# bdsaglam/torch-scae

Measured on AMD Instinct MI355X. Metric: images/sec SCAE fwd+bwd, MNIST 40x40 bs=128, 1/2/4/8 MI355X, higher is better.
Workload: dtype f32

## Files before the change

### include/scae_hip.h

```cpp
#ifndef SCAE_HIP_H
#define SCAE_HIP_H

#include <stdint.h>

#ifdef __cplusplus
extern "C" {
#endif

#define SCAE_ABI_VERSION 3

#define SCAE_OK 0
#define SCAE_ERR_BAD_ARG (-1)
#define SCAE_ERR_UNSUPPORTED (-2)

#define SCAE_MAX_CHANNELS 4
#define SCAE_ATTN_MAX_SET 64
#define SCAE_RENDER_MAX_TEMPLATE_ELEMS 4096

int scae_abi_version(void);
const char *scae_error_string(int code);

void *scae_launch_list_begin(void *stream);
int scae_launch_list_end(void *list);
int scae_launch_list_size(const void *list);
// ... 512 lines not shown

typedef struct scae_batch_source_desc {
  const void *images;
  const void *labels;
  const int32_t *index;
  int64_t rows;
  int64_t n;
  int image_u8, label_u8;
  int C, h, w, H, W;
  int shuffle, translate;
  uint64_t seed;
  int64_t epoch, position;
  int rank, world;
  int wrap;
  const int32_t *affine;
  int64_t affine_rows;
} scae_batch_source_desc;
int scae_gather_batch_f32(float *dst_image, int64_t *dst_label, int B,
                          const scae_batch_source_desc *src, void *stream);
int scae_step_prologue_source_f32(float *dst_image, int64_t *dst_label, int B,
                                  const scae_batch_source_desc *src, float *noise,
                                  int64_t n_noise, uint64_t *noise_state,
                                  const scae_seed_fold_desc *fold,
                                  const scae_first_layer_desc *first, void *stream);

int scae_template_color_supported(int M, int C, int F, int H1);
int scae_template_color_partial_rows(int B, int M);
int scae_template_color_fwd_f32(const float *logits, const float *feature, const float *w1,
                                const float *b1, const float *w2, const float *b2, float *raw,
                                float *templates, float *color, int B, int M, int C, int hw,
                                int F, int H1, int template_nonlin, int color_nonlin,
                                void *stream);
int scae_template_color_bwd_f32(const float *logits, const float *feature, const float *w1,
                                const float *b1, const float *w2, const float *b2,
                                const float *color, const float *g_templates,
                                const float *g_raw, float *g_logits, float *g_feature,
                                float *partial, int B, int M, int C, int hw, int F, int H1,
                                int template_nonlin, int color_nonlin, void *stream);

typedef struct scae_sum_segment {
  float *dst;
  int64_t begin, end, period;
} scae_sum_segment;
int scae_sum_rows_f32(const float *src, int64_t rows, int64_t cols,
                      const scae_sum_segment *segments, int n_segments, void *stream);
typedef struct scae_sum_job {
  const float *src;
  int64_t rows, cols;
  const scae_sum_segment *segments;
  int n_segments;
} scae_sum_job;
int scae_sum_rows_multi_f32(const scae_sum_job *jobs, int n_jobs, void *stream);

typedef struct scae_scaled_sum {
  const float *src;
  int64_t n;
  float scale;
  float *dst;
} scae_scaled_sum;
int scae_scaled_sums_f32(const scae_scaled_sum *jobs, int n_jobs, void *stream);

int scae_capsule_votes_fwd_f32(const float *all_param, const float *cpr_static,
                               const float *bias_cvr, const float *bias_caps,
                               const float *bias_vote, const float *bias_scale,
                               const float *noise_caps, const float *noise_vote,
                               float noise_scale, float *vote, float *scale,
                               float *vote_presence, float *logit_caps,
                               float *logit_vote, float *reg_partial,
                               float *caps_presence, int *caps_arg, int B, int O, int V,
                               int ld_param, int similarity, int learn_vote_scale,
                               int allow_deformations, void *stream);
int scae_capsule_votes_bwd_f32(const float *all_param, const float *cpr_static,
                               const float *bias_cvr, const float *bias_caps,
                               const float *bias_vote, const float *bias_scale,
                               const float *noise_caps, const float *noise_vote,
                               float noise_scale, const float *gvote,
                               const float *gscale, const float *gvote_presence,
                               const float *glogit_caps, const float *glogit_vote,
                               const float *greg, const float *gcaps_presence,
                               const int *caps_arg, float *gall_param, float *gcpr_in,
                               float *gall_param_gated, int B, int O, int V, int ld_param,
                               int similarity, int learn_vote_scale,
                               int allow_deformations, void *stream);

int scae_capsule_likelihood_fwd_f32(
    const float *vote, const float *scale, const float *vote_presence,
    const float *dummy_vote, const float *x, const float *presence,
    float *log_prob_per_point, float *vote_presence_binary, float *winner,
    float *winner_presence, int64_t *winner_idx, int64_t *is_from_capsule,
    float *soft_winner, float *soft_winner_presence, float *posterior,
    float *mixing_log_prob, float *mixing_logit, int B, int O, int M,
    void *stream);
int scae_capsule_likelihood_bwd_f32(
    const float *vote, const float *scale, const float *vote_presence,
    const float *dummy_vote, const float *x, const float *presence,
    const float *posterior, const int64_t *winner_idx, const float *g_lpp,
    const float *g_winner, const float *g_winner_presence,
    const float *g_soft_winner, const float *g_soft_winner_presence,
    const float *g_posterior, const float *g_mixing_log_prob,
    const float *g_mixing_logit, float *gvote, float *gscale,
    float *gvote_presence, float *gx, float *gpresence, float *gdummy_partial,
    int B, int O, int M, void *stream);

int scae_class_probs_supported(int O, int ncls);
int scae_class_probs_f32(const float *caps_presence, const float *posterior, const float *w,
                         const float *bias, float *prior_prob, float *post_prob, int B, int O,
                         int M, int ncls, const scae_scaled_sum *extra_sums, int n_extra,
                         void *stream);

typedef struct scae_eval_sink {
  float *rows;
  int64_t capacity;
  int64_t cursor;
  int64_t overflow;
} scae_eval_sink;
#define SCAE_EVAL_RECORD_FLOATS 9
#define SCAE_EVAL_RECORDS_MAX_CLASSES 64
typedef struct scae_eval_records {
  float *rows;
  int64_t capacity;
  int64_t cursor;
  int64_t overflow;
  int64_t *confusion;
  int64_t ncls;
  int64_t labelled;
} scae_eval_records;
#define SCAE_TRAIN_LOG_ROW 19
typedef struct scae_train_log_desc {
  float *rows;
  int64_t *step;
  int capacity;
  double *acc;
  const float *prior_prob, *post_prob;
  const int64_t *label;
  int ncls;
  const float *lr;
} scae_train_log_desc;
typedef struct scae_loss_extras {
  const float *rec_sums;
  int n_rec;
  const float *reg;
  float w_reg;
  float *g_rec_sums, *g_reg;
  float *loss;
  const float *g_loss;
  int defer_combine;
  float *out12;
  const scae_train_log_desc *train_log;
} scae_loss_extras;
int scae_loss_tail_supported(int B, int O, int ncls);
int64_t scae_loss_tail_workspace_floats(int B, int O, int ncls);
int scae_loss_tail_fwd_f32(const float *lpp, const float *posterior,
                           const float *caps_presence, const float *cls_w,
                           const float *cls_b, const int64_t *label,
                           const scae_loss_extras *extras, float *out12, float *workspace,
                           int B, int O, int M, int ncls, int n_classes_cfg, int prior_type,
                           int post_type, int sparsity_on, const float *weights5,
                           float within_const, void *stream);
int scae_loss_tail_defer_preferred(int B, int O);
int scae_loss_tail_combine_f32(const float *lpp, const float *posterior,
                               const float *caps_presence, const float *cls_w,
                               const float *cls_b, const int64_t *label,
                               const scae_loss_extras *extras, float *out12, float *workspace,
                               int B, int O, int M, int ncls, int n_classes_cfg, int prior_type,
                               int post_type, int sparsity_on, const float *weights5,
                               float within_const, void *stream);
int scae_loss_tail_fwd_class_probs_f32(
    const float *lpp, const float *posterior, const float *caps_presence, const float *cls_w,
    const float *cls_b, const int64_t *label, const scae_loss_extras *extras, float *out12,
    float *workspace, int B, int O, int M, int ncls, int n_classes_cfg, int prior_type,
    int post_type, int sparsity_on, const float *weights5, float within_const,
    const float *cp_caps_presence, const float *cp_posterior, const float *cp_w,
    const float *cp_bias, float *prior_prob, float *post_prob, int cp_B, int cp_O, int cp_M,
    int cp_ncls, const scae_scaled_sum *extra_sums, int n_extra, void *stream);
int scae_loss_tail_fwd_class_probs_sink_f32(
    const float *lpp, const float *posterior, const float *caps_presence, const float *cls_w,
    const float *cls_b, const int64_t *label, const scae_loss_extras *extras, float *out12,
    float *workspace, int B, int O, int M, int ncls, int n_classes_cfg, int prior_type,
    int post_type, int sparsity_on, const float *weights5, float within_const,
    const float *cp_caps_presence, const float *cp_posterior, const float *cp_w,
    const float *cp_bias, float *prior_prob, float *post_prob, int cp_B, int cp_O, int cp_M,
    int cp_ncls, const scae_scaled_sum *extra_sums, int n_extra, scae_eval_sink *sink,
    void *stream);
int scae_loss_tail_bwd_f32(const float *lpp, const float *posterior,
                           const float *caps_presence, const float *cls_w,
                           const float *cls_b, const int64_t *label,
                           const scae_loss_extras *extras, const float *gout12,
                           const float *workspace, float *g_lpp, float *g_posterior,
                           float *g_caps_presence, float *g_cls_w,
                           float *g_cls_b, int B, int O, int M, int ncls, int n_classes_cfg,
                           int prior_type, int post_type, int sparsity_on,
                           const float *weights5, float within_const, void *stream);

#define SCAE_EVAL_ACC_DOUBLES 17
int scae_eval_tail_f32(const float *lpp, const float *posterior, const float *caps_presence,
                       const float *cls_w, const float *cls_b, const int64_t *label,
                       const scae_loss_extras *extras, float *out12, float *workspace, int B,
                       int O, int M, int ncls, int n_classes_cfg, int prior_type,
                       int post_type, int sparsity_on, const float *weights5,
                       float within_const, const float *prior_prob, const float *post_prob,
                       double *acc, float *batch3, void *stream);
int scae_eval_tail_sink_f32(const float *lpp, const float *posterior, const float *caps_presence,
                            const float *cls_w, const float *cls_b, const int64_t *label,
                            const scae_loss_extras *extras, float *out12, float *workspace,
                            int B, int O, int M, int ncls, int n_classes_cfg, int prior_type,
                            int post_type, int sparsity_on, const float *weights5,
                            float within_const, const float *prior_prob, const float *post_prob,
                            double *acc, float *batch3, scae_eval_sink *sink, void *stream);
int scae_eval_tail_records_f32(const float *lpp, const float *posterior,
                               const float *caps_presence, const float *cls_w,
                               const float *cls_b, const int64_t *label,
                               const scae_loss_extras *extras, float *out12, float *workspace,
                               int B, int O, int M, int ncls, int n_classes_cfg, int prior_type,
                               int post_type, int sparsity_on, const float *weights5,
                               float within_const, const float *prior_prob,
                               const float *post_prob, double *acc, float *batch3,
                               scae_eval_sink *sink, scae_eval_records *records, void *stream);
int scae_eval_records_f32(const float *prior_prob, const float *post_prob, const int64_t *label,
                          const float *lpp, const float *rec_sums, const float *rec_pixels,
                          int B, int ncls, int M, int n_rec, scae_eval_records *records,
                          void *stream);
int scae_eval_accumulate_f32(const float *loss, const float *out12, const float *prior_prob,
                             const float *post_prob, const int64_t *label, int B, int ncls,
                             double *acc, float *batch3, void *stream);
int scae_eval_features_f32(const float *caps_presence, const float *posterior, int B, int O,
                           int M, scae_eval_sink *sink, void *stream);
int scae_train_log_f32(const float *loss, const float *out12, const float *extra2,
                       const scae_train_log_desc *log, int B, void *stream);

typedef struct scae_decoder_desc {
  const float *templates;
  const float *templates_alpha;
  const float *pose;
  const float *presence;
  const float *bg_image;
  const float *bg_value;
  const float *bg_mixing_logit;
  const float *temperature_logit;
  const float *out_scale;
  int B, M, C, th, tw, H, W;
  int template_repeat;
} scae_decoder_desc;

int scae_template_render_fwd_f32(const scae_decoder_desc *d,
                                 float *transformed_templates,
                                 float *mixing_logits, void *stream);

int scae_render_gmm_logprob_fwd_f32(const scae_decoder_desc *d, const float *x,
                                    float *log_prob, float *lse_post,
                                    float *lse_prior, void *stream);

int scae_render_gmm_bwd_f32(const scae_decoder_desc *d, const float *x,
                            const float *lse_post, const float *lse_prior,
                            const float *g_logprob, const float *g_tt,
                            const float *g_ml, float *g_templates,
                            float *g_alpha_partial, float *g_pose,
                            float *g_presence, float *g_bg_image,
                            float *g_scalar_partial, void *stream);
int scae_render_gmm_logprob_tiles(const scae_decoder_desc *d);
int scae_render_gmm_logprob_sums_fwd_f32(const scae_decoder_desc *d, const float *x,
                                         float *tile_sums, float *lse_post, float *lse_prior,
                                         void *stream);
int scae_render_gmm_sums_bwd_f32(const scae_decoder_desc *d, const float *x,
                                 const float *lse_post, const float *lse_prior,
                                 const float *g_tile_sums, float *g_templates,
                                 float *g_alpha_partial, float *g_pose, float *g_presence,
                                 float *g_bg_image, float *g_scalar_partial, void *stream);
#define SCAE_K1_FWD_WAVE 0
#define SCAE_K1_FWD_CLASSIC 1
#define SCAE_K1_RENDER_WAVE 0
#define SCAE_K1_RENDER_CLASSIC 1
#define SCAE_K1_BWD_CELL 0
#define SCAE_K1_BWD_SCATTER 1
#define SCAE_K1_BWD_GATHER 2
int scae_render_gmm_forms(const scae_decoder_desc *d, int fused, const void *tt,
                          const void *ml, int out[12]);


int scae_set_encoder_fwd_logprob_f32(int nseg, const float *const *seg_ptr,
                                     const int *seg_width, const int *seg_row_stride,
                                     const int64_t *seg_batch_stride, const float *presence,
                                     const float *params, float *z, float *hsave, int B, int N,
                                     int D, int Din, int Dout, int L, int layer_norm,
                                     const scae_decoder_desc *d, const float *x,
                                     float *tile_sums, float *lse_post, float *lse_prior,
                                     void *stream);

int scae_set_encoder_fwd_logprob_bf16(int nseg, const float *const *seg_ptr,
                                      const int *seg_width, const int *seg_row_stride,
                                      const int64_t *seg_batch_stride, const float *presence,
                                      const float *params, float *z, float *hsave, int B, int N,
                                      int D, int Din, int Dout, int L, int layer_norm,
                                      const scae_decoder_desc *d, const float *x,
                                      float *tile_sums, float *lse_post, float *lse_prior,
                                      void *stream);

typedef struct scae_likelihood_bwd_desc {
  const float *vote, *scale, *vote_presence, *dummy_vote, *x, *presence, *posterior;
  const int64_t *winner_idx;
  const float *g_lpp, *g_winner, *g_winner_presence, *g_soft_winner, *g_soft_winner_presence,
      *g_posterior, *g_mixing_log_prob, *g_mixing_logit;
  float *gvote, *gscale, *gvote_presence, *gx, *gpresence, *gdummy_partial;
  int B, O, M;
} scae_likelihood_bwd_desc;
int scae_render_gmm_sums_bwd_likelihood_f32(
    const scae_decoder_desc *d, const float *x, const float *lse_post, const float *lse_prior,
    const float *g_tile_sums, float *g_templates, float *g_alpha_partial, float *g_pose,
    float *g_presence, float *g_bg_image, float *g_scalar_partial,
    const scae_likelihood_bwd_desc *k, void *stream);

int scae_gmm_log_prob_fwd_f32(const float *loc, const float *mixing_logits,
                              const float *sigma, const float *x,
                              float *log_prob, int B, int K, int C, int Cm,
                              int64_t P, void *stream);
int scae_gmm_log_prob_bwd_f32(const float *loc, const float *mixing_logits,
                              const float *sigma, const float *x,
                              const float *g_logprob, float *g_loc,
                              float *g_ml, float *g_sigma_partial, float *g_x,
                              int B, int K, int C, int Cm, int64_t P,
                              void *stream);
int scae_gmm_mean_f32(const float *loc, const float *mixing_logits, float *out,
                      int B, int K, int C, int Cm, int64_t P, void *stream);
int scae_gmm_mode_f32(const float *loc, const float *mixing_logits,
                      const float *sigma, float *out, int maximum, int B,
                      int K, int C, int Cm, int64_t P, void *stream);

int scae_render_gmm_mode_f32(const scae_decoder_desc *d, float *out, int what, int first,
                             int count, void *stream);

int scae_render_gmm_parts_f32(const scae_decoder_desc *d, const float *x, const int *part_group,
                              const float *palette, int P, int *part, float *conf, float *mass,
                              float *mass_partial, int *group, float *rgb_part,
                              float *rgb_group, int first, int count, void *stream);
int scae_render_gmm_parts_geometry(const scae_decoder_desc *d, int count, int *out);

int scae_image_sheet_f32(int nsrc, const float *const *src, const int *n, int C, int H, int W,
                         int nrow, int padding, float pad_value, float *sheet, void *stream);

#define SCAE_KMEANS_MAX_K 256
#define SCAE_KMEANS_MAX_F 256
#define SCAE_KMEANS_MAX_KF 16384
#define SCAE_KMEANS_STATE_INTS 4
int scae_kmeans_supported(int k, int F);
int scae_kmeans_groups(int64_t N, int R);
typedef struct scae_kmeans_desc {
  const float *x;
  int64_t N;
  int F, k, R;
  int G;
  int max_iter;
  float *centroids;
  int64_t *labels;
  float *part_sum;
  int *part_count;
  int *part_changed;
  double *part_inertia;
  int *state;
  double *inertia;
} scae_kmeans_desc;
int scae_kmeans_lloyd_f32(const scae_kmeans_desc *d, int n_iters, void *stream);
int scae_kmeans_pp_f32(const float *x, int64_t N, int F, int k, int R, uint32_t seed,
                       float *centroids, float *d2, int64_t *chosen, void *stream);
int scae_kmeans_assign_f32(const float *x, int64_t N, int F, int k, const float *centroids,
                           int64_t *labels, void *stream);
int scae_kmeans_contingency(const int64_t *cluster_ids, const int64_t *labels, int64_t N, int k,
                            int ncls, int *table, int *outside, void *stream);

#define SCAE_PROBE_MAX_F 256
#define SCAE_PROBE_MAX_C 256
#define SCAE_PROBE_MAX_CF 16384
#define SCAE_PROBE_MAX_R 16
#define SCAE_PROBE_STATE_INTS 4
int scae_probe_supported(int F, int C, int R);
int scae_probe_groups(int64_t N, int F);
int scae_probe_predict_blocks(int64_t N);
int scae_probe_moments_f64(const float *x, const int64_t *y, int64_t N, int F, int C,
                           double *part, double *moments, int *outside, void *stream);
typedef struct scae_probe_desc {
  const float *x;
  const int64_t *y;
  int64_t N;
  int F, C, R;
  int G;
  int max_iter;
  const float *mean;
  const float *scale;
  const double *l2;
  const double *step;
  const double *tol;
  float *W, *V;
  float *grad;
  double *t;
  float *part_grad;
  double *part_loss;
  double *history;
  int *state;
} scae_probe_desc;
int scae_probe_fit_f32(const scae_probe_desc *d, int n_iters, void *stream);
int scae_probe_predict_f32(const float *x, int64_t N, int F, int C, const float *weight,
                           const float *bias, const int64_t *y, int64_t *pred, float *log_prob,
                           double *part_ce, double *mean_ce, void *stream);

#define SCAE_TSNE_MAX_N 32768
#define SCAE_TSNE_MAX_F 256
#define SCAE_TSNE_HISTORY_COLS 3
#define SCAE_TSNE_BLOCK_DOUBLES 640
int scae_tsne_supported(int N, int F);
int scae_tsne_groups(int N);
int scae_tsne_affinities_f32(const float *x, int N, int F, float perplexity, float *P,
                             float *beta, double *part, double *plogp, void *stream);
typedef struct scae_tsne_desc {
  int N;
  int G;
  int n_iter;
  int exaggeration_iter;
  int check_every;
  float early_exaggeration;
  float learning_rate;
  const float *P;
  float *Y, *velocity, *gains;
  float *part;
  float *rows;
  double *block;
  const double *plogp;
  double *history;
} scae_tsne_desc;
int scae_tsne_run_f32(const scae_tsne_desc *d, int first_iter, int n, void *stream);

#define SCAE_KNN_MAX_K 64
#define SCAE_KNN_MAX_F 256
#define SCAE_KNN_MAX_KS 8
int scae_knn_supported(int64_t Nq, int64_t Nb, int F, int k);
int scae_knn_groups(int64_t Nq, int64_t Nb);
int scae_knn_f32(const float *q, int64_t Nq, const float *base, int64_t Nb, int F, int k,
                 int self_mode, uint64_t *part, float *d2, int64_t *idx, void *stream);
int scae_knn_vote_f32(const int64_t *idx, const float *d2, int64_t Nq, int k,
                      const int64_t *base_labels, int64_t Nb, const int *ks, int n_ks,
                      int weighted, int64_t *pred, void *stream);
int scae_knn_ranks_f32(const float *x, int64_t N, int F, const int64_t *idx, int k, int *rank,
                       int *part_count, int64_t *part, int64_t *penalty, void *stream);

#define SCAE_TSNE_MAX_NEIGHBORS 128
#define SCAE_TSNE_SPARSE_MAX_N 262144
#define SCAE_TSNE_SPARSE_BLOCK_DOUBLES 5120
int scae_knn_wide_f32(const float *x, int64_t N, int F, int k, uint64_t *part, float *d2,
                      int64_t *idx, void *stream);
int scae_tsne_sparse_supported(int N, int F, int K);
int scae_tsne_sparse_groups(int N);
int scae_tsne_knn_bandwidths_f32(const float *d2, int N, int K, float perplexity, float *cond,
                                 float *beta, void *stream);
typedef struct scae_tsne_sparse_desc {
  int N;
  int G;
  int n_iter;
  int exaggeration_iter;
  int check_every;
  float early_exaggeration;
  float learning_rate;
  const int64_t *indptr;
  const int *cols;
  const float *vals;
  int64_t nnz;
  float *Y, *velocity, *gains;
  float *part;
  float *rows;
  double *block;
  const double *plogp;
  double *history;
} scae_tsne_sparse_desc;
int scae_tsne_sparse_run_f32(const scae_tsne_sparse_desc *d, int first_iter, int n, void *stream);

#define SCAE_CLUSTER_QUALITY_MAX_F 256
int scae_cluster_quality_supported(int64_t N, int F, int64_t k);
int scae_cluster_quality_labels(const int64_t *labels, int64_t N, int64_t k, int *lab32,
                                int *outside, void *stream);
int scae_cluster_quality_silhouette_f32(const float *xs, const int *ls, const int64_t *off,
                                        const int64_t *order, int64_t N, int F, int64_t k,
                                        double *values, double *a, double *b, int64_t *nearest,
                                        double *sorted_values, double *scores, void *stream);
int scae_cluster_quality_dispersion_f32(const float *xs, const int64_t *off, int64_t N, int F,
                                        int64_t k, double *table, void *stream);

#ifdef __cplusplus
}
#endif
#endif
```

### torch_scae_amd/_lib.py

```python
import ctypes
import os
from ctypes import c_float

from . import _abi

_HERE = os.path.dirname(os.path.abspath(__file__))
LIB_PATH = os.environ.get("SCAE_HIP_LIB") or os.path.join(_HERE, "lib",
                                                        "libscae_hip.so")
HEADER_PATH = os.path.join(os.path.dirname(_HERE), "include", "scae_hip.h")

DEVICE_STRUCTS = {"scae_eval_sink", "scae_eval_records"}


class ScaeHipError(RuntimeError):
    pass


def _read_header():
    if not os.path.exists(HEADER_PATH):
        raise ScaeHipError(
            f"{HEADER_PATH} is missing: the binding is derived from it, and torch_scae_amd "
            "runs from its source tree (restore the file, e.g. `git checkout "
            "include/scae_hip.h`).")
    with open(HEADER_PATH) as f:
        return _abi.parse(f.read(), by_address=DEVICE_STRUCTS)


ABI = _read_header()
SIGNATURES = {name: p.argtypes for name, p in ABI.prototypes.items()}
globals().update({cls.__name__: cls for cls in ABI.structs.values()})
globals().update({name[len("SCAE_"):]: value for name, value in ABI.defines.items()})
ABI_VERSION = ABI.defines["SCAE_ABI_VERSION"]
ERR_UNSUPPORTED = ABI.defines["SCAE_ERR_UNSUPPORTED"]

EVAL_SINK_INT64S = ctypes.sizeof(ABI.structs["scae_eval_sink"]) // 8
EVAL_RECORDS_INT64S = ctypes.sizeof(ABI.structs["scae_eval_records"]) // 8
assert (EVAL_SINK_INT64S, EVAL_RECORDS_INT64S) == (4, 7)
assert all(ctypes.sizeof(t) == 8 for name in DEVICE_STRUCTS
           for _, t in ABI.structs[name]._fields_)

_lib = None


def load():
    global _lib
    if _lib is not None:
        return _lib
    if not os.path.exists(LIB_PATH):
        raise ScaeHipError(
            f"{LIB_PATH} is missing: build it with `python -c 'import "
            f"__graft_entry__ as g; g.build()'` or `make -C torch_scae_amd/csrc`."
            " torch_scae_amd has no CPU / eager fallback.")
    lib = ctypes.CDLL(LIB_PATH)
    for name, proto in ABI.prototypes.items():
        fn = getattr(lib, name)
        fn.argtypes = proto.argtypes
        fn.restype = proto.restype
        if _is_launcher(proto):
            setattr(lib, name, _recording(fn))
    if lib.scae_abi_version() != ABI_VERSION:
        raise ScaeHipError(
            f"{LIB_PATH} has ABI version {lib.scae_abi_version()}, {HEADER_PATH} "
            f"declares version {ABI_VERSION}: rebuild it (make -C torch_scae_amd/csrc)")
    _lib = lib
    return lib


_RECORDER = None


def _is_launcher(proto):
    return (bool(proto.decls) and proto.decls[-1] == "void *stream"
            and not proto.name.startswith("scae_launch_list"))


def _recording(fn):
    def launcher(*args):
        rc = fn(*args)
        if _RECORDER is not None and rc == 0:
            conv = []
            for t, a in zip(fn.argtypes, args):
                if a is None or isinstance(a, (int, float)):
                    a = t(a) if a is not None else t()
                conv.append(a)
            _RECORDER.append((fn, tuple(conv[:-1]), args))
        return rc
    launcher.__name__ = getattr(fn, "__name__", "launcher")
    return launcher


class recorder:

    def __enter__(self):
        global _RECORDER
        self.prev, self.launches = _RECORDER, []
        _RECORDER = self.launches
        return self.launches

    def __exit__(self, *exc):
        global _RECORDER
        _RECORDER = self.prev
        return False


def replay(launches, stream):
    for fn, cargs, _keep in launches:
        rc = fn(*cargs, stream)
        if rc != 0:
            check(rc, getattr(fn, "__name__", "launch"))


def check(rc, what):
    if rc != 0:
        msg = load().scae_error_string(rc)
        raise ScaeHipError(f"{what} failed with code {rc}: "
                           f"{msg.decode() if msg else '?'}")


def call(name, *args):
    check(getattr(load(), name)(*args), name)


def try_call(name, *args):
    rc = getattr(load(), name)(*args)
    if rc == ERR_UNSUPPORTED:
        return False
    check(rc, name)
    return True
```

### torch_scae_amd/csrc/capsule_votes.hip

```cpp
#include "common.h"

#include "capsule_votes_dev.h"

namespace {
using namespace scae_votes;
constexpr int NT = 64;

__global__ __launch_bounds__(NT) void votes_fwd_kernel(
    VoteArgs a, float *__restrict__ vote, float *__restrict__ scale,
    float *__restrict__ vote_presence, float *__restrict__ logit_caps,
    float *__restrict__ logit_vote, float *__restrict__ reg_partial,
    float *__restrict__ caps_presence, int *__restrict__ caps_arg) {
  const int bo = blockIdx.x, o = bo % a.O, V = a.V, lane = threadIdx.x;
  const float *ap = a.all_param + (size_t)bo * a.ldp;

  float cv[6];
#pragma unroll
  for (int i = 0; i < 6; ++i) cv[i] = ap[6 * V + i] + a.bias_cvr[o * 6 + i];
  Xf C;
  xf_eval(cv, a.similarity, C);

  float lc = ap[6 * V + 6] + a.bias_caps[o];
  if (a.noise_caps) lc += (a.noise_caps[bo] - 0.5f) * a.noise_scale;
  const float pc = scae::sigmoidf_(lc);
  if (lane == 0) logit_caps[bo] = lc;

  float reg = 0.f;
  float best = -INFINITY;
  int best_v = 0x7fffffff;
  for (int v = lane; v < V; v += NT) {
    float pr[6];
#pragma unroll
    for (int i = 0; i < 6; ++i) {
      float dyn = a.allow_deformations ? ap[v * 6 + i] : 0.f;
      reg += dyn * dyn;
      pr[i] = dyn + a.cpr_static[((size_t)o * V + v) * 6 + i];
    }
    Xf P;
    xf_eval(pr, a.similarity, P);
    float *vo = vote + ((size_t)bo * V + v) * 6;
    vo[0] = C.o[0] * P.o[0] + C.o[1] * P.o[3];
    vo[1] = C.o[0] * P.o[1] + C.o[1] * P.o[4];
    vo[2] = C.o[0] * P.o[2] + C.o[1] * P.o[5] + C.o[2];
    vo[3] = C.o[3] * P.o[0] + C.o[4] * P.o[3];
    vo[4] = C.o[3] * P.o[1] + C.o[4] * P.o[4];
    vo[5] = C.o[3] * P.o[2] + C.o[4] * P.o[5] + C.o[5];

    float lv = ap[6 * V + 7 + v] + a.bias_vote[o * V + v];
    if (a.noise_vote) lv += (a.noise_vote[(size_t)bo * V + v] - 0.5f) * a.noise_scale;
    logit_vote[(size_t)bo * V + v] = lv;
    const float vpv = pc * scae::sigmoidf_(lv);
    vote_presence[(size_t)bo * V + v] = vpv;
    if (vpv > best) best = vpv, best_v = v;
    float sc = 1.f;
    if (a.learn_vote_scale)
      sc = scae::softplusf_(ap[7 * V + 7 + v] + a.bias_scale[o * V + v] + .5f) + 1e-2f;
    scale[(size_t)bo * V + v] = sc;
  }
  reg = scae::wave_sum(reg);
  if (lane == 0) reg_partial[bo] = reg;
  if (caps_presence) {
#pragma unroll
    for (int off = 32; off > 0; off >>= 1) {
      const float ov = __shfl_xor(best, off, 64);
      const int oi = __shfl_xor(best_v, off, 64);
      if (ov > best || (ov == best && oi < best_v)) best = ov, best_v = oi;
    }
    if (lane == 0) {
      caps_presence[bo] = best;
      caps_arg[bo] = best_v;
    }
  }
}

__global__ __launch_bounds__(NT) void votes_bwd_kernel(
    VoteArgs a, const float *__restrict__ gvote, const float *__restrict__ gscale,
    const float *__restrict__ gvp, const float *__restrict__ glc,
    const float *__restrict__ glv, const float *__restrict__ greg,
    float *__restrict__ gall, float *__restrict__ gcpr_in,
    const float *__restrict__ g_caps_presence, const int *__restrict__ caps_arg,
    float *__restrict__ gall_gated) {
  const int bo = blockIdx.x, o = bo % a.O, V = a.V, lane = threadIdx.x;
  const float *ap = a.all_param + (size_t)bo * a.ldp;
  float *ga = gall + (size_t)bo * a.ldp;
  float *gg = gall_gated ? gall_gated + (size_t)bo * a.ldp : nullptr;
  auto put = [&](int i, float v) {
    ga[i] = v;
    if (gg) gg[i] = ap[i] > 0.f ? v : 0.f;
  };

  float cv[6];
#pragma unroll
  for (int i = 0; i < 6; ++i) cv[i] = ap[6 * V + i] + a.bias_cvr[o * 6 + i];
  Xf C;
  xf_eval(cv, a.similarity, C);
  float lc = ap[6 * V + 6] + a.bias_caps[o];
  if (a.noise_caps) lc += (a.noise_caps[bo] - 0.5f) * a.noise_scale;
  const float pc = scae::sigmoidf_(lc);
  const float reg_w = greg ? greg[0] / (float)a.B : 0.f;

  float gC[6] = {0, 0, 0, 0, 0, 0};
  float gpc = 0.f;
  for (int v = lane; v < V; v += NT) {
    float pr[6], dyn[6];
#pragma unroll
    for (int i = 0; i < 6; ++i) {
      dyn[i] = a.allow_deformations ? ap[v * 6 + i] : 0.f;
      pr[i] = dyn[i] + a.cpr_static[((size_t)o * V + v) * 6 + i];
    }
    Xf P;
    xf_eval(pr, a.similarity, P);
    float gv[6] = {0, 0, 0, 0, 0, 0};
    if (gvote) {
#pragma unroll
      for (int i = 0; i < 6; ++i) gv[i] = gvote[((size_t)bo * V + v) * 6 + i];
    }
    gC[0] += gv[0] * P.o[0] + gv[1] * P.o[1] + gv[2] * P.o[2];
    gC[1] += gv[0] * P.o[3] + gv[1] * P.o[4] + gv[2] * P.o[5];
    gC[2] += gv[2];
    gC[3] += gv[3] * P.o[0] + gv[4] * P.o[1] + gv[5] * P.o[2];
    gC[4] += gv[3] * P.o[3] + gv[4] * P.o[4] + gv[5] * P.o[5];
    gC[5] += gv[5];
    float gP[6];
    gP[0] = gv[0] * C.o[0] + gv[3] * C.o[3];
    gP[1] = gv[1] * C.o[0] + gv[4] * C.o[3];
    gP[2] = gv[2] * C.o[0] + gv[5] * C.o[3];
    gP[3] = gv[0] * C.o[1] + gv[3] * C.o[4];
    gP[4] = gv[1] * C.o[1] + gv[4] * C.o[4];
    gP[5] = gv[2] * C.o[1] + gv[5] * C.o[4];
    float gin[6];
    xf_backward(P, a.similarity, gP, gin);
#pragma unroll
    for (int i = 0; i < 6; ++i) {
      gcpr_in[((size_t)bo * V + v) * 6 + i] = gin[i];
      put(v * 6 + i, a.allow_deformations ? gin[i] + reg_w * dyn[i] : 0.f);
    }

    float lv = ap[6 * V + 7 + v] + a.bias_vote[o * V + v];
    if (a.noise_vote) lv += (a.noise_vote[(size_t)bo * V + v] - 0.5f) * a.noise_scale;
    const float pv = scae::sigmoidf_(lv);
    float g_vp = gvp ? gvp[(size_t)bo * V + v] : 0.f;
    if (g_caps_presence && caps_arg[bo] == v) g_vp += g_caps_presence[bo];
    gpc += g_vp * pv;
    float g_lv = g_vp * pc * pv * (1.f - pv);
    if (glv) g_lv += glv[(size_t)bo * V + v];
    put(6 * V + 7 + v, g_lv);
    float g_sc = 0.f;
    if (a.learn_vote_scale && gscale)
      g_sc = gscale[(size_t)bo * V + v] *
             scae::softplus_grad(ap[7 * V + 7 + v] + a.bias_scale[o * V + v] + .5f);
    put(7 * V + 7 + v, g_sc);
  }
#pragma unroll
  for (int i = 0; i < 6; ++i) gC[i] = scae::wave_sum(gC[i]);
  gpc = scae::wave_sum(gpc);
  if (lane == 0) {
    float gin[6];
    xf_backward(C, a.similarity, gC, gin);
#pragma unroll
    for (int i = 0; i < 6; ++i) put(6 * V + i, gin[i]);
    float g_lc = gpc * pc * (1.f - pc);
    if (glc) g_lc += glc[bo];
    put(6 * V + 6, g_lc);
  }
}

int check_votes(const VoteArgs &a) {
  if (!a.all_param || !a.cpr_static || !a.bias_cvr || !a.bias_caps || !a.bias_vote ||
      !a.bias_scale)
    return SCAE_ERR_BAD_ARG;
  if (a.B <= 0 || a.O <= 0 || a.V <= 0 || a.ldp < 8 * a.V + 7) return SCAE_ERR_BAD_ARG;
  return SCAE_OK;
}
}

extern "C" int scae_capsule_votes_fwd_f32(
    const float *all_param, const float *cpr_static, const float *bias_cvr,
    const float *bias_caps, const float *bias_vote, const float *bias_scale,
    const float *noise_caps, const float *noise_vote, float noise_scale, float *vote,
    float *scale, float *vote_presence, float *logit_caps, float *logit_vote,
    float *reg_partial, float *caps_presence, int *caps_arg, int B, int O, int V,
    int ld_param, int similarity, int learn_vote_scale, int allow_deformations, void *stream) {
  VoteArgs a{all_param, cpr_static, bias_cvr, bias_caps, bias_vote, bias_scale,
             noise_caps, noise_vote, noise_scale, B, O, V, similarity, learn_vote_scale,
             allow_deformations, ld_param > 0 ? ld_param : 8 * V + 7};
  int rc = check_votes(a);
  if (rc) return rc;
  SCAE_REQUIRE(vote && scale && vote_presence && logit_caps && logit_vote && reg_partial);
  SCAE_REQUIRE(!caps_presence == !caps_arg);
  scae::launch(votes_fwd_kernel, dim3(B * O), dim3(NT), 0, (hipStream_t)stream, a,
                     vote, scale, vote_presence, logit_caps, logit_vote, reg_partial,
                     caps_presence, caps_arg);
  return scae_launch_status();
}

extern "C" int scae_capsule_votes_bwd_f32(
    const float *all_param, const float *cpr_static, const float *bias_cvr,
    const float *bias_caps, const float *bias_vote, const float *bias_scale,
    const float *noise_caps, const float *noise_vote, float noise_scale,
    const float *gvote, const float *gscale, const float *gvote_presence,
    const float *glogit_caps, const float *glogit_vote, const float *greg,
    const float *gcaps_presence, const int *caps_arg, float *gall_param, float *gcpr_in,
    float *gall_param_gated, int B, int O, int V, int ld_param, int similarity,
    int learn_vote_scale, int allow_deformations, void *stream) {
  VoteArgs a{all_param, cpr_static, bias_cvr, bias_caps, bias_vote, bias_scale,
             noise_caps, noise_vote, noise_scale, B, O, V, similarity, learn_vote_scale,
             allow_deformations, ld_param > 0 ? ld_param : 8 * V + 7};
  int rc = check_votes(a);
  if (rc) return rc;
  SCAE_REQUIRE(gall_param && gcpr_in && (!gcaps_presence || caps_arg));
  scae::launch(votes_bwd_kernel, dim3(B * O), dim3(NT), 0, (hipStream_t)stream, a,
                     gvote, gscale, gvote_presence, glogit_caps, glogit_vote, greg,
                     gall_param, gcpr_in, gcaps_presence, caps_arg, gall_param_gated);
  return scae_launch_status();
}
```

### torch_scae_amd/csrc/capsule_votes_dev.h

```cpp
#pragma once
#include "common.h"

namespace scae_votes {
constexpr float kTwoPi = 6.283185307179586f;

struct Xf {
  float sx, sy, sh, c, s, tx, ty;
  float dsx, dsy, dsh, dtx, dty;
  float o[6];
};

__device__ __forceinline__ void xf_eval(const float *p, int similarity, Xf &g) {
  const float ex = scae::sigmoidf_(p[0]), ey = scae::sigmoidf_(p[1]);
  g.sx = ex + 1e-2f;
  g.sy = ey + 1e-2f;
  g.dsx = ex * (1.f - ex);
  g.dsy = ey * (1.f - ey);
  g.sh = tanhf(p[3] * 5.f);
  g.tx = tanhf(p[4] * 5.f);
  g.ty = tanhf(p[5] * 5.f);
  g.dsh = 5.f * (1.f - g.sh * g.sh);
  g.dtx = 5.f * (1.f - g.tx * g.tx);
  g.dty = 5.f * (1.f - g.ty * g.ty);
  const float th = p[2] * kTwoPi;
  g.c = cosf(th);
  g.s = sinf(th);
  if (similarity) {
    g.o[0] = g.sx * g.c;
    g.o[1] = -g.sx * g.s;
    g.o[2] = g.tx;
    g.o[3] = g.sx * g.s;
    g.o[4] = g.sx * g.c;
    g.o[5] = g.ty;
  } else {
    g.o[0] = g.sx * g.c + g.sh * g.sy * g.s;
    g.o[1] = -g.sx * g.s + g.sh * g.sy * g.c;
    g.o[2] = g.tx;
    g.o[3] = g.sy * g.s;
    g.o[4] = g.sy * g.c;
    g.o[5] = g.ty;
  }
}

__device__ __forceinline__ void xf_backward(const Xf &g, int similarity, const float *go,
                                            float *gp) {
  float gsx, gsy, gsh, gth;
  if (similarity) {
    gsx = go[0] * g.c - go[1] * g.s + go[3] * g.s + go[4] * g.c;
    gsy = 0.f;
    gsh = 0.f;
    gth = g.sx * (-go[0] * g.s - go[1] * g.c + go[3] * g.c - go[4] * g.s);
  } else {
    gsx = go[0] * g.c - go[1] * g.s;
    gsy = go[0] * g.sh * g.s + go[1] * g.sh * g.c + go[3] * g.s + go[4] * g.c;
    gsh = go[0] * g.sy * g.s + go[1] * g.sy * g.c;
    gth = go[0] * (-g.sx * g.s + g.sh * g.sy * g.c) +
          go[1] * (-g.sx * g.c - g.sh * g.sy * g.s) + go[3] * g.sy * g.c - go[4] * g.sy * g.s;
  }
  gp[0] = gsx * g.dsx;
  gp[1] = gsy * g.dsy;
  gp[2] = gth * kTwoPi;
  gp[3] = gsh * g.dsh;
  gp[4] = go[2] * g.dtx;
  gp[5] = go[5] * g.dty;
}

struct VoteArgs {
  const float *all_param, *cpr_static, *bias_cvr, *bias_caps, *bias_vote, *bias_scale;
  const float *noise_caps, *noise_vote;
  float noise_scale;
  int B, O, V, similarity, learn_vote_scale, allow_deformations;
  int ldp;
};


struct VoteOut {
  float *vote, *scale, *vote_presence, *logit_caps, *logit_vote, *reg_partial, *caps_presence;
  int *caps_arg;
};
struct VoteGrads {
  const float *gvote, *gscale, *gvp, *glc, *glv, *greg, *g_caps_presence;
  const int *caps_arg;
  float *gall, *gcpr_in, *gall_gated;
};

template <int NTH>
__device__ __forceinline__ void fwd_block(const VoteArgs &a, const VoteOut &w, const float *rows,
                                          int ld, float *red, int b0, int o) {
  const int V = a.V, tid = threadIdx.x;
  for (int e = tid; e < 16 * V; e += NTH) {
    const int i = e / V, v = e - i * V, b = b0 + i;
    const float *ap = rows + i * ld;
    float regv = 0.f, vpv = -INFINITY;
    if (b < a.B) {
      const int bo = b * a.O + o;
      float cv[6];
#pragma unroll
      for (int k = 0; k < 6; ++k) cv[k] = ap[6 * V + k] + a.bias_cvr[o * 6 + k];
      Xf C;
      xf_eval(cv, a.similarity, C);
      float lc = ap[6 * V + 6] + a.bias_caps[o];
      if (a.noise_caps) lc += (a.noise_caps[bo] - 0.5f) * a.noise_scale;
      const float pc = scae::sigmoidf_(lc);
      if (v == 0) w.logit_caps[bo] = lc;
      float pr[6];
#pragma unroll
      for (int k = 0; k < 6; ++k) {
        const float dyn = a.allow_deformations ? ap[v * 6 + k] : 0.f;
        regv += dyn * dyn;
        pr[k] = dyn + a.cpr_static[((size_t)o * V + v) * 6 + k];
      }
      Xf P;
      xf_eval(pr, a.similarity, P);
      float *vo = w.vote + ((size_t)bo * V + v) * 6;
      vo[0] = C.o[0] * P.o[0] + C.o[1] * P.o[3];
      vo[1] = C.o[0] * P.o[1] + C.o[1] * P.o[4];
      vo[2] = C.o[0] * P.o[2] + C.o[1] * P.o[5] + C.o[2];
      vo[3] = C.o[3] * P.o[0] + C.o[4] * P.o[3];
      vo[4] = C.o[3] * P.o[1] + C.o[4] * P.o[4];
      vo[5] = C.o[3] * P.o[2] + C.o[4] * P.o[5] + C.o[5];
      float lv = ap[6 * V + 7 + v] + a.bias_vote[o * V + v];
      if (a.noise_vote) lv += (a.noise_vote[(size_t)bo * V + v] - 0.5f) * a.noise_scale;
      w.logit_vote[(size_t)bo * V + v] = lv;
      vpv = pc * scae::sigmoidf_(lv);
      w.vote_presence[(size_t)bo * V + v] = vpv;
      float sc = 1.f;
      if (a.learn_vote_scale)
        sc = scae::softplusf_(ap[7 * V + 7 + v] + a.bias_scale[o * V + v] + .5f) + 1e-2f;
      w.scale[(size_t)bo * V + v] = sc;
    }
    red[e] = regv;
    red[16 * V + e] = vpv;
  }
  __syncthreads();
  if (tid < 256) {
    const int i = tid >> 4, l = tid & 15;
    float reg = 0.f, best = -INFINITY;
    int best_v = 0x7fffffff;
    for (int v = l; v < V; v += 16) {
      reg += red[i * V + v];
      const float p = red[16 * V + i * V + v];
      if (p > best) best = p, best_v = v;
    }
#pragma unroll
    for (int off = 8; off > 0; off >>= 1) {
      reg += __shfl_xor(reg, off, 64);
      const float ov = __shfl_xor(best, off, 64);
      const int oi = __shfl_xor(best_v, off, 64);
      if (ov > best || (ov == best && oi < best_v)) best = ov, best_v = oi;
    }
    if (l == 0 && b0 + i < a.B) {
      const int bo = (b0 + i) * a.O + o;
      w.reg_partial[bo] = reg;
      if (w.caps_presence) {
        w.caps_presence[bo] = best;
        w.caps_arg[bo] = best_v;
      }
    }
  }
}

template <int NTH>
__device__ __forceinline__ void bwd_block(const VoteArgs &a, const VoteGrads &w, float *grows,
                                          int ld, float *red, int b0, int o) {
  const int V = a.V, tid = threadIdx.x, A = 8 * V + 7;
  const float reg_w = w.greg ? w.greg[0] / (float)a.B : 0.f;
  auto put = [&](const float *ap, int i, int bo, int col, float v) {
    w.gall[(size_t)bo * a.ldp + col] = v;
    const float gv = ap[col] > 0.f ? v : 0.f;
    if (w.gall_gated) w.gall_gated[(size_t)bo * a.ldp + col] = gv;
    grows[i * ld + col] = w.gall_gated ? gv : v;
  };
  for (int e = tid; e < 16 * V; e += NTH) {
    const int i = e / V, v = e - i * V, b = b0 + i;
    float part[7] = {0.f, 0.f, 0.f, 0.f, 0.f, 0.f, 0.f};
    if (b < a.B) {
      const int bo = b * a.O + o;
      const float *ap = a.all_param + (size_t)bo * a.ldp;
      float cv[6];
#pragma unroll
      for (int k = 0; k < 6; ++k) cv[k] = ap[6 * V + k] + a.bias_cvr[o * 6 + k];
      Xf C;
      xf_eval(cv, a.similarity, C);
      float lc = ap[6 * V + 6] + a.bias_caps[o];
      if (a.noise_caps) lc += (a.noise_caps[bo] - 0.5f) * a.noise_scale;
      const float pc = scae::sigmoidf_(lc);
      float pr[6], dyn[6];
#pragma unroll
      for (int k = 0; k < 6; ++k) {
        dyn[k] = a.allow_deformations ? ap[v * 6 + k] : 0.f;
        pr[k] = dyn[k] + a.cpr_static[((size_t)o * V + v) * 6 + k];
      }
      Xf P;
      xf_eval(pr, a.similarity, P);
      float gv[6] = {0, 0, 0, 0, 0, 0};
      if (w.gvote) {
#pragma unroll
        for (int k = 0; k < 6; ++k) gv[k] = w.gvote[((size_t)bo * V + v) * 6 + k];
      }
      part[0] = gv[0] * P.o[0] + gv[1] * P.o[1] + gv[2] * P.o[2];
      part[1] = gv[0] * P.o[3] + gv[1] * P.o[4] + gv[2] * P.o[5];
      part[2] = gv[2];
      part[3] = gv[3] * P.o[0] + gv[4] * P.o[1] + gv[5] * P.o[2];
      part[4] = gv[3] * P.o[3] + gv[4] * P.o[4] + gv[5] * P.o[5];
      part[5] = gv[5];
      float gP[6];
      gP[0] = gv[0] * C.o[0] + gv[3] * C.o[3];
      gP[1] = gv[1] * C.o[0] + gv[4] * C.o[3];
      gP[2] = gv[2] * C.o[0] + gv[5] * C.o[3];
      gP[3] = gv[0] * C.o[1] + gv[3] * C.o[4];
      gP[4] = gv[1] * C.o[1] + gv[4] * C.o[4];
      gP[5] = gv[2] * C.o[1] + gv[5] * C.o[4];
      float gin[6];
      xf_backward(P, a.similarity, gP, gin);
#pragma unroll
      for (int k = 0; k < 6; ++k) {
        w.gcpr_in[((size_t)bo * V + v) * 6 + k] = gin[k];
        put(ap, i, bo, v * 6 + k, a.allow_deformations ? gin[k] + reg_w * dyn[k] : 0.f);
      }
      float lv = ap[6 * V + 7 + v] + a.bias_vote[o * V + v];
      if (a.noise_vote) lv += (a.noise_vote[(size_t)bo * V + v] - 0.5f) * a.noise_scale;
      const float pv = scae::sigmoidf_(lv);
      float g_vp = w.gvp ? w.gvp[(size_t)bo * V + v] : 0.f;
      if (w.g_caps_presence && w.caps_arg[bo] == v) g_vp += w.g_caps_presence[bo];
      part[6] = g_vp * pv;
      float g_lv = g_vp * pc * pv * (1.f - pv);
      if (w.glv) g_lv += w.glv[(size_t)bo * V + v];
      put(ap, i, bo, 6 * V + 7 + v, g_lv);
      float g_sc = 0.f;
      if (a.learn_vote_scale && w.gscale)
        g_sc = w.gscale[(size_t)bo * V + v] *
               scae::softplus_grad(ap[7 * V + 7 + v] + a.bias_scale[o * V + v] + .5f);
      put(ap, i, bo, 7 * V + 7 + v, g_sc);
    }
#pragma unroll
    for (int k = 0; k < 7; ++k) red[(size_t)e * 7 + k] = part[k];
  }
  __syncthreads();
  {
    float t = 0.f;
    const int i = tid >> 5, k = (tid >> 2) & 7, part = tid & 3;
    if (tid < 512 && k < 7)
      for (int v = part; v < V; v += 4) t += red[(size_t)(i * V + v) * 7 + k];
    t += __shfl_xor(t, 1, 64);
    t += __shfl_xor(t, 2, 64);
    __syncthreads();
    if (tid < 512 && k < 7 && part == 0) red[i * 8 + k] = t;
  }
  __syncthreads();
  if (tid < 16) {
    const int i = tid, b = b0 + i;
    if (b < a.B) {
      const int bo = b * a.O + o;
      const float *ap = a.all_param + (size_t)bo * a.ldp;
      float gC[6], gpc = red[i * 8 + 6];
#pragma unroll
      for (int k = 0; k < 6; ++k) gC[k] = red[i * 8 + k];
      float cv[6];
#pragma unroll
      for (int k = 0; k < 6; ++k) cv[k] = ap[6 * V + k] + a.bias_cvr[o * 6 + k];
      Xf C;
      xf_eval(cv, a.similarity, C);
      float lc = ap[6 * V + 6] + a.bias_caps[o];
      if (a.noise_caps) lc += (a.noise_caps[bo] - 0.5f) * a.noise_scale;
      const float pc = scae::sigmoidf_(lc);
      float gin[6];
      xf_backward(C, a.similarity, gC, gin);
#pragma unroll
      for (int k = 0; k < 6; ++k) put(ap, i, bo, 6 * V + k, gin[k]);
      float g_lc = gpc * pc * (1.f - pc);
      if (w.glc) g_lc += w.glc[bo];
      put(ap, i, bo, 6 * V + 6, g_lc);
    } else {
      for (int col = 0; col < A; ++col) grows[i * ld + col] = 0.f;
    }
  }
  const int a16 = (A + 15) & ~15;
  for (int e = tid; e < 16 * (a16 - A); e += NTH) {
    const int i = e / (a16 - A), col = A + e - i * (a16 - A);
    grows[i * ld + col] = 0.f;
  }
  __syncthreads();
}
}
```

### torch_scae_amd/csrc/render_bwd_likelihood.hip

```cpp
#include "common.h"
#include "capsule_likelihood_dev.h"
#include "render_gmm_wave_dev.h"

namespace {
struct LkBwd {
  scae_lk::LkArgs a;
  const int64_t *winner_idx;
  const float *g_lpp, *g_winner, *g_winner_presence, *g_soft_winner, *g_soft_winner_presence,
      *g_posterior, *g_mlp, *g_mlogit;
  float *gvote, *gscale, *gvp, *gx, *gpresence, *gdummy;
};

template <int C>
__global__ __launch_bounds__(256, 5) void bwd_cell_likelihood_kernel(
    scae_decoder_desc d, const float *__restrict__ x, const float *__restrict__ lse_post,
    const float *__restrict__ lse_prior, const float *__restrict__ g_tile, int lp_tiles,
    int lp_ppb, float *__restrict__ g_templates, float *__restrict__ g_alpha_partial,
    float *__restrict__ g_pose, float *__restrict__ g_presence, float *__restrict__ g_bg_image,
    float *__restrict__ g_scalar_partial, int chunk_rows, int max_items, int item_budget,
    LkBwd lk, int n_lk) {
  extern __shared__ __attribute__((aligned(16))) float smem[];
  if ((int)blockIdx.x < n_lk) {
    scae_lk::likelihood_bwd_body<false, 256>(
        lk.a, lk.winner_idx, lk.g_lpp, lk.g_winner, lk.g_winner_presence, lk.g_soft_winner,
        lk.g_soft_winner_presence, lk.g_posterior, lk.g_mlp, lk.g_mlogit, lk.gvote, lk.gscale,
        lk.gvp, lk.gx, lk.gpresence, lk.gdummy, smem, blockIdx.x, n_lk);
    return;
  }
  const int id = (int)blockIdx.x - n_lk, K = d.M + 1, b = id / K, k = id - b * K;
  scae_k1::bwd_cell_body<C, 256>(d, x, lse_post, lse_prior, nullptr, g_tile, lp_tiles, lp_ppb,
                                 g_templates, g_alpha_partial, g_pose, g_presence, g_bg_image,
                                 g_scalar_partial, chunk_rows, max_items, item_budget, smem, k, b);
}

template <int C>
int launch(const scae_decoder_desc *d, const scae_k1::CellGeom &g, const scae_k1::LpTiling &lt,
           const float *x, const float *lse_post, const float *lse_prior, const float *g_tile,
           float *g_templates, float *g_alpha_partial, float *g_pose, float *g_presence,
           float *g_bg_image, float *g_scalar_partial, const LkBwd &lk, hipStream_t st) {
  const size_t lds_k = scae_lk::lk_lds(lk.a.O, lk.a.M, true);
  const size_t lds = g.lds > lds_k ? g.lds : lds_k;
  if (lds > 48 * 1024) {
    hipError_t e =
        hipFuncSetAttribute(reinterpret_cast<const void *>(bwd_cell_likelihood_kernel<C>),
                            hipFuncAttributeMaxDynamicSharedMemorySize, (int)lds);
    if (e != hipSuccess) return (int)e;
  }
  const int n_lk = lk.a.B < 1024 ? lk.a.B : 1024;
  scae::launch((bwd_cell_likelihood_kernel<C>), dim3(n_lk + (d->M + 1) * d->B), dim3(256),
                     lds, st, *d, x, lse_post, lse_prior, g_tile, lt.tiles, lt.ppb, g_templates,
                     g_alpha_partial, g_pose, g_presence, g_bg_image, g_scalar_partial,
                     g.chunk_rows, g.max_items, g.item_budget, lk, n_lk);
  return scae_launch_status();
}
}

extern "C" int scae_render_gmm_sums_bwd_likelihood_f32(
    const scae_decoder_desc *d, const float *x, const float *lse_post, const float *lse_prior,
    const float *g_tile_sums, float *g_templates, float *g_alpha_partial, float *g_pose,
    float *g_presence, float *g_bg_image, float *g_scalar_partial,
    const scae_likelihood_bwd_desc *k, void *stream) {
  SCAE_REQUIRE(d && k);
  const char *e = getenv("SCAE_FUSE_K1_K4_BWD");
  const scae_k1::CellGeom g = scae_k1::cell_geom(d);
  const bool fits = !(e && *e == '0') && g.lds && (d->C == 1 || d->C == 3) && k->O <= 64 &&
                    scae_lk::lk_lds(k->O, k->M, true) <= g.lds && k->B > 0 && k->O > 0 &&
                    k->M > 0 && d->template_repeat <= 1;
  if (!fits) {
    int rc = scae_render_gmm_sums_bwd_f32(d, x, lse_post, lse_prior, g_tile_sums, g_templates,
                                          g_alpha_partial, g_pose, g_presence, g_bg_image,
                                          g_scalar_partial, stream);
    if (rc) return rc;
    return scae_capsule_likelihood_bwd_f32(
        k->vote, k->scale, k->vote_presence, k->dummy_vote, k->x, k->presence, k->posterior,
        k->winner_idx, k->g_lpp, k->g_winner, k->g_winner_presence, k->g_soft_winner,
        k->g_soft_winner_presence, k->g_posterior, k->g_mixing_log_prob, k->g_mixing_logit,
        k->gvote, k->gscale, k->gvote_presence, k->gx, k->gpresence, k->gdummy_partial, k->B,
        k->O, k->M, stream);
  }
  SCAE_REQUIRE(x && lse_post && lse_prior && g_tile_sums && g_templates && g_alpha_partial &&
               g_pose && g_scalar_partial);
  SCAE_REQUIRE(k->vote && k->scale && k->vote_presence && k->dummy_vote && k->x &&
               k->posterior && k->winner_idx && k->gvote && k->gscale && k->gvote_presence &&
               k->gx && k->gdummy_partial);
  const scae_k1::LpTiling lt = scae_k1::lp_tiling(d);
  LkBwd lk{{k->vote, k->scale, k->vote_presence, k->dummy_vote, k->x, k->presence, k->B, k->O,
            k->M},
           k->winner_idx,
           k->g_lpp,
           k->g_winner,
           k->g_winner_presence,
           k->g_soft_winner,
           k->g_soft_winner_presence,
           k->g_posterior,
           k->g_mixing_log_prob,
           k->g_mixing_logit,
           k->gvote,
           k->gscale,
           k->gvote_presence,
           k->gx,
           k->gpresence,
           k->gdummy_partial};
  hipStream_t st = (hipStream_t)stream;
  return d->C == 1 ? launch<1>(d, g, lt, x, lse_post, lse_prior, g_tile_sums, g_templates,
                               g_alpha_partial, g_pose, g_presence, g_bg_image, g_scalar_partial,
                               lk, st)
                   : launch<3>(d, g, lt, x, lse_post, lse_prior, g_tile_sums, g_templates,
                               g_alpha_partial, g_pose, g_presence, g_bg_image, g_scalar_partial,
                               lk, st);
}
```

### torch_scae_amd/ops.py

```python
import collections
import ctypes
import functools

import numpy as np
import torch

from . import _lib, step_plan
from ._lib import DecoderDesc, ScaeHipError
from .step_plan import StepPlan, current as _plan

__all__ = ["geometric_transform", "qkv_attention", "set_encoder", "grouped_mlp", "seed_attention", "seed_attention_supported", "seed_fold", "seed_fold_supported", "loss_tail", "loss_tail_scalar", "loss_tail_supported", "capsule_votes",
           "capsule_likelihood", "colored_templates", "template_color_supported", "attention_conv_pool", "attention_pool_supported", "capsule_head", "part_encoder", "conv_stack", "conv_stack_supported",
           "uniform", "reset_noise", "pack_params", "render_templates", "render_gmm_log_prob", "render_gmm_log_prob_sums",
           "gmm_log_prob", "gmm_mean", "gmm_mode", "render_gmm_mode", "render_gmm_parts", "GmmParts", "image_sheet", "ScaeHipError"]


def _need_hip(*tensors):
    for t in tensors:
        if t is None:
            continue
        if not t.is_cuda:
            raise ScaeHipError(
                "torch_scae_amd ops run only on a HIP device (got a "
                f"{t.device} tensor); there is no CPU path.")
# ... 1790 lines not shown
            gy2 = gy2.contiguous()
        gw = _grad_out(ctx.slots[0], weight)
        gb = _grad_out(ctx.slots[1], weight, (N,)) if ctx.has_bias else None
        wgrad = _gemm_desc(_p(gy2), _p(x2), _p(gw), 1, N, K, M, False, N, 0,
                           False, K, 0, K, 0, asum=_p(gb), asum_b=0, asum_ld=1)
        if ctx.needs_input_grad[0]:
            gx = torch.empty(M, K, device=x2.device, dtype=x2.dtype)
            dgrad = _gemm_desc(_p(gy2), _p(weight), _p(gx), 1, M, K, N, True, N,
                               0, False, K, 0, K, 0)
            _gemm_pair(wgrad, dgrad, x2)
            gx = gx.view(ctx.x_shape)
        else:
            gx = None
            _lib.call("scae_gemm_multi_f32", (_lib.GemmDesc * 1)(wgrad), 1,
                      _stream(x2))
        return gx, gw, gb


def linear(x, weight, bias=None):
    return _Linear.apply(x, weight, bias)


class HipLinear(torch.nn.Linear):

    def forward(self, x):
        if x.is_cuda and x.dtype == torch.float32 and \
                self.weight.dtype == torch.float32 and not _bf16() and \
                not torch.is_autocast_enabled("cuda"):
            return linear(x, self.weight, self.bias)
        return torch.nn.functional.linear(x, self.weight, self.bias)


class _LayerNorm(torch.autograd.Function):

    @_fwd
    def forward(ctx, x, weight, bias, eps):
        _need_hip(x, weight, bias)
        d = x.shape[-1]
        x2 = x.reshape(-1, d).contiguous()
        rows = x2.shape[0]
        y = torch.empty_like(x2)
        mean = torch.empty(rows, device=x.device, dtype=x.dtype)
        rstd = torch.empty_like(mean)
        _lib.call("scae_layer_norm_fwd_f32", _p(x2), _p(_c(weight)),
                  _p(_c(bias)), _p(y), _p(mean), _p(rstd), rows, d, float(eps),
                  _stream(x))
        ctx.save_for_backward(x2, mean, rstd, *([weight] if weight is not None
                                                else []))
        ctx.has = (weight is not None, bias is not None)
        ctx.x_shape = x.shape
        ctx.slots = (_slot(weight, ctx) if weight is not None else None,
                     _slot(bias, ctx) if bias is not None else None)
        return y.view(x.shape)

    @_bwd
    def backward(ctx, gy):
        x2, mean, rstd = ctx.saved_tensors[:3]
        weight = ctx.saved_tensors[3] if ctx.has[0] else None
        rows, d = x2.shape
        gy2 = gy.reshape(rows, d).contiguous()
        gx = torch.empty_like(x2) if ctx.needs_input_grad[0] else None
        want_p = ctx.has[0] or ctx.has[1]
        partial = torch.empty(_lib.load().scae_layer_norm_rows(rows), 2 * d,
                              device=x2.device, dtype=x2.dtype) \
            if want_p else None
        _lib.call("scae_layer_norm_bwd_f32", _p(x2), _p(_c(weight)), _p(mean),
                  _p(rstd), _p(gy2), _p(gx), _p(partial), rows, d, _stream(x2))
        gw = gb = None
        if want_p:
            outs = [_grad_out(ctx.slots[0], x2, (d,)) if ctx.has[0] else
                    torch.empty(d, device=x2.device, dtype=x2.dtype),
                    _grad_out(ctx.slots[1], x2, (d,)) if ctx.has[1] else
                    torch.empty(d, device=x2.device, dtype=x2.dtype)]
            gw, gb = _sum_rows(partial, [(d,), (d,)], outs=outs)
            gw = gw if ctx.has[0] else None
            gb = gb if ctx.has[1] else None
        return (None if gx is None else gx.view(ctx.x_shape)), gw, gb, None


class HipLayerNorm(torch.nn.LayerNorm):

    def forward(self, x):
        if x.is_cuda and x.dtype == torch.float32 and \
                len(self.normalized_shape) == 1 and \
                self.normalized_shape[0] <= 1024 and \
                not torch.is_autocast_enabled("cuda"):
            return _LayerNorm.apply(x, self.weight, self.bias, self.eps)
        return super().forward(x)


def mlp_chain_supported(x, layers):
    if not x.is_cuda or x.dtype != torch.float32 or \
            not 1 <= len(layers) <= 4:
        return False
    wmax = _lib.load().scae_mlp_chain_max_width()
    return x.shape[2] <= wmax and all(
        w.shape[1] <= wmax and w.shape[2] <= wmax + 1 and
        not (ones and b is not None) for w, b, ones in layers)


def _chain_forward_desc(x, ones_flags, weights, biases):
    L = len(ones_flags)
    B, G, Kin = x.shape
    d = _lib.MlpChainDesc()
    d.n_layers, d.in_, d.in_gs, d.in_bs, d.in_dim, d.B, d.G = \
        L, x.data_ptr(), x.stride(1), x.stride(0), Kin, B, G
    d.row_tile = _CHAIN_ROW_TILE
    d.bf16 = int(_bf16())
    acts, K = [], Kin
    for l, (w, b) in enumerate(zip(weights, biases)):
        N, ldw = w.shape[1], w.shape[2]
        assert ldw == K + (1 if ones_flags[l] else 0)
        if l == L - 1:
            Np = (N + 3) // 4 * 4
            out = torch.empty(B, G, Np, device=x.device,
                              dtype=x.dtype)[:, :, :N]
            out_gs, out_bs = Np, G * Np
        else:
            out = torch.empty(G, B, N, device=x.device, dtype=x.dtype)
            out_gs, out_bs = B * N, N
        y = d.layer[l]
        y.w, y.w_gs, y.ldw, y.K, y.N = w.data_ptr(), N * ldw, ldw, K, N
        if ones_flags[l]:
            y.bias, y.bias_gs, y.bias_ld = w.data_ptr() + 4 * K, N * ldw, ldw
        elif b is not None:
            y.bias, y.bias_gs, y.bias_ld = b.data_ptr(), N, 1
        y.out, y.out_gs, y.out_bs, y.relu = out.data_ptr(), out_gs, out_bs, 1
        acts.append(out)
        K = N
    return d, acts


_CHAIN_ROW_TILE = 0


def _chain_backward(x, weights, acts, ones_flags, has_bias, x_is_relu, slots,
                    need_gx, gpre=None, votes=None, park=False):
    L = len(ones_flags)
    B, G, Kin = x.shape
    dev, dt = x.device, x.dtype
    d = _lib.MlpChainDesc()
    d.n_layers, d.in_, d.in_gs, d.in_bs, d.in_dim, d.B, d.G = \
        L, gpre.data_ptr(), gpre.stride(1), gpre.stride(0), gpre.shape[2], B, G
    d.row_tile = _CHAIN_ROW_TILE
    d.bf16 = int(_bf16())
    gx = torch.empty(B, G, Kin, device=dev, dtype=dt) if need_gx else None
    gs = [None] * L
    gs[L - 1] = gpre
    n_chain = 0
    for i, l in enumerate(range(L - 1, -1, -1)):
        w = weights[l]
        N, ldw = w.shape[1], w.shape[2]
        K = ldw - (1 if ones_flags[l] else 0)
        if l == 0 and not need_gx:
            break
        y = d.layer[i]
        y.w, y.w_gs, y.ldw, y.K, y.N = w.data_ptr(), N * ldw, ldw, N, K
        if l > 0:
            gs[l - 1] = torch.empty(G, B, K, device=dev, dtype=dt)
            y.gate, y.gate_gs, y.gate_bs = acts[l - 1].data_ptr(), B * K, K
            y.out, y.out_gs, y.out_bs = gs[l - 1].data_ptr(), B * K, K
        else:
            if x_is_relu:
                y.gate, y.gate_gs, y.gate_bs = x.data_ptr(), x.stride(1), \
                    x.stride(0)
            y.out, y.out_gs, y.out_bs = gx.data_ptr(), K, G * K
        n_chain += 1
    d.n_layers = n_chain
    if votes is not None:
        assert n_chain >= 1
        _lib.call("scae_mlp_chain_votes_bwd_f32", ctypes.byref(d),
                  ctypes.byref(votes), _stream(x))
    elif n_chain:
        _lib.call("scae_mlp_chain_bwd_f32", ctypes.byref(d), _stream(x))
    descs = (_lib.GemmDesc * L)()
    gws, gbs = [None] * L, [None] * L
    for l in range(L):
        w = weights[l]
        N, ldw = w.shape[1], w.shape[2]
        K = ldw - (1 if ones_flags[l] else 0)
        if l == 0:
            xin, x_ld, x_b = x, x.stride(0), x.stride(1)
        else:
            xin, x_ld, x_b = acts[l - 1], K, B * K
        g = gs[l]
        if l == L - 1:
            g_ld, g_b = g.stride(0), g.stride(1)
        else:
            g_ld, g_b = N, B * N
        gw = _grad_out(slots[l], w)
        asum_ld = 1
        if has_bias[l]:
            gsum = _grad_out(slots[L + l], w, (G, N))
            asum, asum_b = _p(gsum), N
            gbs[l] = gsum
        elif ones_flags[l]:
            asum, asum_b, asum_ld = _off(gw, K), N * ldw, ldw
        else:
            asum, asum_b = None, 0
        descs[l] = _gemm_desc(_p(g), _p(xin), _p(gw), G, N, K, B, False,
                              g_ld, g_b, False, x_ld, x_b, ldw, N * ldw,
                              asum=asum, asum_b=asum_b, asum_ld=asum_ld)
        gws[l] = gw
    if park and not _bf16() and L <= 4 and all(_in_slot(t) for t in gws) and \
            all(_in_slot(t) for t in gbs if t is not None):
        _plan().park("wgrads", _PendingWeightGemms(
            descs, L, (x, gs, acts, [w for w in weights]), x))
    else:
        _lib.call(_prec("scae_gemm_multi_f32"), descs, L, _stream(x))
    return gx, gws, gbs


class _MLPChain(torch.autograd.Function):

    @_fwd
    def forward(ctx, x, ones_flags, x_is_relu, *wb):
        L = len(ones_flags)
        _need_hip(x, *wb)
        if x.stride(2) != 1:
            x = x.contiguous()
        weights = [w.contiguous() for w in wb[:L]]
        biases = [None if b is None else b.contiguous() for b in wb[L:]]
        d, acts = _chain_forward_desc(x, ones_flags, weights, biases)
        _lib.call("scae_mlp_chain_fwd_f32", ctypes.byref(d), _stream(x))
        ctx.save_for_backward(x, *weights, *acts)
        ctx.meta = (tuple(ones_flags), [b is not None for b in biases],
                    bool(x_is_relu))
        ctx.slots = [_slot(t, ctx) for t in wb]
        return acts[-1]

    @_bwd
    def backward(ctx, gy):
        ones_flags, has_bias, x_is_relu = ctx.meta
        L = len(ones_flags)
        x = ctx.saved_tensors[0]
        weights = ctx.saved_tensors[1:1 + L]
        acts = ctx.saved_tensors[1 + L:]
        G = x.shape[1]
        gpre = gy
        if not (gpre.stride(2) == 1 and gpre.stride(1) >= gpre.shape[2]
                and gpre.stride(0) == G * gpre.stride(1)):
            gpre = gpre.contiguous()
        gx, gws, gbs = _chain_backward(x, weights, acts, ones_flags, has_bias,
                                       x_is_relu, ctx.slots,
                                       ctx.needs_input_grad[0], gpre=gpre)
        return (gx, None, None, *gws, *gbs)


class _ChainVotes(torch.autograd.Function):

    @_fwd
    def forward(ctx, x, ones_flags, vflags, noise_scale, cpr_static, b_cvr,
                b_caps, b_vote, b_scale, noise_caps, noise_vote, *wb):
        L = len(ones_flags)
        similarity, learn_vote_scale, allow_deformations, defer_reg = vflags
        _need_hip(x, cpr_static, b_cvr, b_caps, b_vote, b_scale, noise_caps,
                  noise_vote, *wb)
        if x.stride(2) != 1:
            x = x.contiguous()
        weights = [w.contiguous() for w in wb[:L]]
        biases = [None if b is None else b.contiguous() for b in wb[L:]]
        vargs = [_c(t) for t in (cpr_static, b_cvr, b_caps, b_vote, b_scale,
                                 noise_caps, noise_vote)]
        d, acts = _chain_forward_desc(x, ones_flags, weights, biases)
        all_param = acts[-1]
        B, O, A = all_param.shape
        V, ldp = (A - 7) // 8, all_param.stride(1)
        assert A == 8 * V + 7
        dev, dt = x.device, x.dtype
        new = lambda *shape: torch.empty(*shape, device=dev, dtype=dt)
        vote, scale, vp = new(B, O, V, 6), new(B, O, V), new(B, O, V)
        lc, lv, reg = new(B, O, 1), new(B, O, V), new(B, O)
        reg_loss = torch.empty((), device=dev, dtype=dt)
        caps_presence = new(B, O)
        caps_arg = torch.empty(B, O, device=dev, dtype=torch.int32)
        v = _lib.VotesDesc()
        for name, t in zip(("cpr_static", "bias_cvr", "bias_caps", "bias_vote",
                            "bias_scale", "noise_caps", "noise_vote"), vargs):
            setattr(v, name, None if t is None else t.data_ptr())
        v.noise_scale, v.V, v.ld_param = float(noise_scale), V, ldp
        v.similarity, v.learn_vote_scale, v.allow_deformations = \
            int(similarity), int(learn_vote_scale), int(allow_deformations)
        for name, t in (("vote", vote), ("scale", scale), ("vote_presence", vp),
                        ("logit_caps", lc), ("logit_vote", lv),
                        ("reg_partial", reg), ("caps_presence", caps_presence),
                        ("caps_arg", caps_arg)):
            setattr(v, name, t.data_ptr())
        _lib.call("scae_mlp_chain_votes_fwd_f32", ctypes.byref(d),
                  ctypes.byref(v), _stream(x))
        if not defer_reg:
            scaled_sums([(reg, 0.5 / B, reg_loss)])
        ctx.save_for_backward(x, caps_arg, *weights, *acts,
                              *[t for t in vargs if t is not None])
        ctx.has_noise = (vargs[5] is not None, vargs[6] is not None)
        ctx.meta = (tuple(ones_flags), [b is not None for b in biases],
                    float(noise_scale), (V, ldp, int(similarity),
                                         int(learn_vote_scale),
                                         int(allow_deformations)))
        ctx.slots = [_slot(t, ctx) for t in wb]
        ctx.vslots = [_slot(t, ctx) for t in (cpr_static, b_cvr, b_caps, b_vote,
                                         b_scale)]
        ctx.set_materialize_grads(False)
        ctx.mark_non_differentiable(reg)
        return vote, scale, vp, lc, lv, reg_loss, caps_presence, reg

    @_bwd
    def backward(ctx, gvote, gscale, gvp, glc, glv, greg, gcp, _greg_partial):
        ones_flags, has_bias, noise_scale, (V, ldp, sim, lvs, adef) = ctx.meta
        L = len(ones_flags)
        saved = list(ctx.saved_tensors)
        x, caps_arg = saved[0], saved[1]
        weights = saved[2:2 + L]
        acts = saved[2 + L:2 + 2 * L]
        rest = saved[2 + 2 * L:]
        vargs = rest[:5]
        rest = rest[5:]
        noise_caps = rest.pop(0) if ctx.has_noise[0] else None
        noise_vote = rest.pop(0) if ctx.has_noise[1] else None
        all_param = acts[-1]
        B, O, A = all_param.shape
        dev, dt = x.device, x.dtype
        padded = lambda: torch.empty(B, O, ldp, device=dev,
                                     dtype=dt)[:, :, :A]
        gall, ggated = padded(), padded()
        gin = torch.empty(B, O, V, 6, device=dev, dtype=dt)
        grads = [_c(g) for g in (gvote, gscale, gvp, glc, glv, greg, gcp)]
        v = _lib.VotesDesc()
        for name, t in zip(("all_param", "cpr_static", "bias_cvr", "bias_caps",
                            "bias_vote", "bias_scale", "noise_caps",
                            "noise_vote"),
                           [all_param, *vargs, noise_caps, noise_vote]):
            setattr(v, name, None if t is None else t.data_ptr())
        v.noise_scale, v.V, v.ld_param = noise_scale, V, ldp
        v.similarity, v.learn_vote_scale, v.allow_deformations = sim, lvs, adef
        for name, t in zip(("gvote", "gscale", "gvote_presence", "glogit_caps",
                            "glogit_vote", "greg", "gcaps_presence"), grads):
            setattr(v, name, None if t is None else t.data_ptr())
        v.caps_arg = caps_arg.data_ptr()
        v.gall_param, v.gcpr_in, v.gall_param_gated = \
            gall.data_ptr(), gin.data_ptr(), ggated.data_ptr()
        gx, gws, gbs = _chain_backward(
            x, weights, acts, ones_flags, has_bias, False, ctx.slots, True,
            gpre=ggated, votes=v,
            park=ctx.plan.parking)
        outs = [_grad_out(sl, t) for sl, t in zip(ctx.vslots, vargs)]
        gall_rows = torch.as_strided(gall, (B, O * ldp), (O * ldp, 1))
        (g_static,), (g_cvr, g_caps, g_vote, g_scale) = _sum_rows_multi([
            dict(partial=gin.view(B, -1), shapes=[vargs[0].shape],
                 outs=outs[:1], defer=ctx.vslots[0] is not None),
            dict(partial=gall_rows, shapes=[t.shape for t in vargs[1:5]],
                 starts=[6 * V, 6 * V + 6, 6 * V + 7, 7 * V + 7], period=ldp,
                 outs=outs[1:],
                 defer=all(sl is not None for sl in ctx.vslots[1:5]))])
        return (gx, None, None, None, g_static, g_cvr, g_caps, g_vote, g_scale,
                None, None, *gws, *gbs)


def chain_votes(x, layers, cpr_static, bias_cvr, bias_caps, bias_vote,
                bias_scale, noise_caps=None, noise_vote=None, noise_scale=0.,
                similarity=False, learn_vote_scale=True,
                allow_deformations=True, defer_reg=False):
    ws = [w for w, _, _ in layers]
    bs = [b for _, b, _ in layers]
    return _ChainVotes.apply(
        x, tuple(bool(o) for _, _, o in layers),
        (bool(similarity), bool(learn_vote_scale), bool(allow_deformations),
         bool(defer_reg)), float(noise_scale), cpr_static, bias_cvr, bias_caps,
        bias_vote, bias_scale, noise_caps, noise_vote, *ws, *bs)


def mlp_chain(x, layers, x_is_relu=False):
    ws = [w for w, _, _ in layers]
    bs = [b for _, b, _ in layers]
    return _MLPChain.apply(x, tuple(bool(o) for _, _, o in layers),
                           bool(x_is_relu), *ws, *bs)


def grouped_mlp(x, weights, biases, ones_input=False, grad_pregated=False,
                x_is_relu=False, pad_out=False):
    biases = list(biases) if biases is not None else [None] * len(weights)
    return _GroupedMLP.apply(x, ones_input, len(weights), grad_pregated,
                             x_is_relu, pad_out, *weights, *biases)


class _CapsuleVotes(torch.autograd.Function):
    @_fwd
    def forward(ctx, all_param, cpr_static, b_cvr, b_caps, b_vote, b_scale,
                noise_caps, noise_vote, noise_scale, similarity,
                learn_vote_scale, allow_deformations, param_is_relu,
                defer_reg):
        _need_hip(all_param, cpr_static, b_cvr, b_caps, b_vote, b_scale,
                  noise_caps, noise_vote)
        B, O, A = all_param.shape
        V = (A - 7) // 8
        ldp = all_param.stride(1)
        if not (all_param.stride(2) == 1 and ldp >= A
                and all_param.stride(0) == O * ldp):
            all_param, ldp = all_param.contiguous(), A
        args = [all_param] + [_c(t) for t in (cpr_static, b_cvr, b_caps, b_vote,
                                              b_scale, noise_caps, noise_vote)]
        dev, dt = all_param.device, all_param.dtype
        vote = torch.empty(B, O, V, 6, device=dev, dtype=dt)
        scale = torch.empty(B, O, V, device=dev, dtype=dt)
        vp = torch.empty(B, O, V, device=dev, dtype=dt)
        lc = torch.empty(B, O, 1, device=dev, dtype=dt)
        lv = torch.empty(B, O, V, device=dev, dtype=dt)
        reg = torch.empty(B, O, device=dev, dtype=dt)
        reg_loss = torch.empty((), device=dev, dtype=dt)
        caps_presence = torch.empty(B, O, device=dev, dtype=dt)
        caps_arg = torch.empty(B, O, device=dev, dtype=torch.int32)
        flags = (B, O, V, ldp, int(similarity), int(learn_vote_scale),
                 int(allow_deformations))
        _lib.call("scae_capsule_votes_fwd_f32", *[_p(t) for t in args],
                  float(noise_scale), _p(vote), _p(scale), _p(vp), _p(lc),
                  _p(lv), _p(reg), _p(caps_presence), _p(caps_arg), *flags,
                  _stream(all_param))
        if not defer_reg:
            scaled_sums([(reg, 0.5 / B, reg_loss)])
        ctx.save_for_backward(caps_arg, *[t for t in args if t is not None])
        ctx.has_noise = (args[6] is not None, args[7] is not None)
        ctx.noise_scale = float(noise_scale)
        ctx.flags = flags
        ctx.param_is_relu = bool(param_is_relu)
        ctx.slots = [_slot(t, ctx) for t in (cpr_static, b_cvr, b_caps, b_vote,
                                        b_scale)]
        ctx.set_materialize_grads(False)
        ctx.mark_non_differentiable(reg)
        return vote, scale, vp, lc, lv, reg_loss, caps_presence, reg

    @_bwd
    def backward(ctx, gvote, gscale, gvp, glc, glv, greg, gcp, _greg_partial):
        saved = list(ctx.saved_tensors)
        caps_arg = saved.pop(0)
        args = saved[:6]
        args.append(saved.pop(6) if ctx.has_noise[0] else None)
        args.append(saved[6] if ctx.has_noise[1] else None)
        all_param = args[0]
        B, O, V, ldp = ctx.flags[:4]
        A = all_param.shape[2]
        padded = lambda: torch.empty(B, O, ldp, device=all_param.device,
                                     dtype=all_param.dtype)[:, :, :A]
        gall = padded()
        ggated = padded() if ctx.param_is_relu else None
        gin = torch.empty(B, O, V, 6, device=all_param.device,
                          dtype=all_param.dtype)
        grads = [_c(g) for g in (gvote, gscale, gvp, glc, glv, greg, gcp)]
        _lib.call("scae_capsule_votes_bwd_f32", *[_p(t) for t in args],
                  ctx.noise_scale, *[_p(g) for g in grads], _p(caps_arg),
                  _p(gall), _p(gin), _p(ggated), *ctx.flags,
                  _stream(all_param))
        outs = [_grad_out(sl, t) for sl, t in zip(ctx.slots, args[1:6])]
        gall_rows = torch.as_strided(gall, (B, O * ldp), (O * ldp, 1))
        (g_static,), (g_cvr, g_caps, g_vote, g_scale) = _sum_rows_multi([
            dict(partial=gin.view(B, -1), shapes=[args[1].shape],
                 outs=outs[:1], defer=ctx.slots[0] is not None),
            dict(partial=gall_rows,
                 shapes=[t.shape for t in args[2:6]],
                 starts=[6 * V, 6 * V + 6, 6 * V + 7, 7 * V + 7], period=ldp,
                 outs=outs[1:],
                 defer=all(sl is not None for sl in ctx.slots[1:5]))])
        return (gall if ggated is None else ggated, g_static, g_cvr, g_caps,
                g_vote, g_scale, None, None, None, None, None, None, None, None)


def capsule_votes(all_param, cpr_static, bias_cvr, bias_caps, bias_vote,
                  bias_scale, noise_caps=None, noise_vote=None, noise_scale=0.,
                  similarity=False, learn_vote_scale=True,
                  allow_deformations=True, param_is_relu=False,
                  defer_reg=False):
    return _CapsuleVotes.apply(all_param, cpr_static, bias_cvr, bias_caps,
                               bias_vote, bias_scale, noise_caps, noise_vote,
                               noise_scale, similarity, learn_vote_scale,
                               allow_deformations, param_is_relu, defer_reg)


class _CapsuleLikelihood(torch.autograd.Function):
    @_fwd
    def forward(ctx, vote, scale, vp, dummy_vote, x, presence, defer_sum):
        _need_hip(vote, scale, vp, dummy_vote, x, presence)
        vote, scale, vp, dummy_vote, x, presence = (
            _c(t) for t in (vote, scale, vp, dummy_vote, x, presence))
        B, O, M, _ = vote.shape
        dev, dt = vote.device, vote.dtype
        f = lambda *s: torch.empty(*s, device=dev, dtype=dt)
        lpp, binary = f(B, M), f(B, O, M)
        winner, winner_p = f(B, M, 6), f(B, M)
        widx = torch.empty(B, M, device=dev, dtype=torch.int64)
        from_caps = torch.empty(B, M, device=dev, dtype=torch.int64)
        soft, soft_p = f(B, M, 6), f(B, M)
        post, mlp, mlogit = f(B, O + 1, M), f(B, O + 1, M), f(B, O + 1, M)
        log_prob = torch.empty((), device=dev, dtype=dt)
        _lib.call("scae_capsule_likelihood_fwd_f32", _p(vote), _p(scale),
                  _p(vp), _p(dummy_vote), _p(x), _p(presence), _p(lpp),
                  _p(binary), _p(winner), _p(winner_p), _p(widx),
                  _p(from_caps), _p(soft), _p(soft_p), _p(post), _p(mlp),
                  _p(mlogit), B, O, M, _stream(vote))
        if not defer_sum:
            scaled_sums([(lpp, 1.0 / B, log_prob)])
        saved = [vote, scale, vp, dummy_vote, x, post, widx]
        if presence is not None:
            saved.append(presence)
        ctx.save_for_backward(*saved)
        ctx.has_presence = presence is not None
        ctx.dims = (B, O, M)
        ctx.dummy_shape = dummy_vote.shape
        ctx.mark_non_differentiable(binary, widx, from_caps)
        ctx.set_materialize_grads(False)
        return (lpp, binary, winner, winner_p, widx, from_caps, soft, soft_p,
                post, mlp, mlogit, log_prob)

    @_bwd
    def backward(ctx, g_lpp, _gb, g_w, g_wp, _gi, _gf, g_s, g_sp, g_post,
                 g_mlp, g_mlogit, g_log_prob):
        saved = ctx.saved_tensors
        vote, scale, vp, dummy_vote, x, post, widx = saved[:7]
        presence = saved[7] if ctx.has_presence else None
        B, O, M = ctx.dims
        if g_log_prob is not None:
            spread = (g_log_prob / B).expand(B, M)
            g_lpp = spread if g_lpp is None else g_lpp + spread
        gvote, gscale, gvp = (torch.empty_like(t) for t in (vote, scale, vp))
        gx = torch.empty_like(x)
        gpres = torch.empty(B, M, device=x.device, dtype=x.dtype) \
            if presence is not None else None
        gdummy = torch.empty(B, M, 6, device=x.device, dtype=x.dtype)
        gin = [_c(g) for g in (g_lpp, g_w, g_wp, g_s, g_sp, g_post, g_mlp,
                               g_mlogit)]
        pending = ctx.plan.take("k1_bwd")
        if pending is not None and any(
                g is not None for g in (g_w, g_wp, g_s, g_sp)):
            pending.launch_alone()
            pending = None
        if pending is not None and pending.ref.device == vote.device:
            k = _lib.LikelihoodBwdDesc()
            for name, t in zip(
                    ("vote", "scale", "vote_presence", "dummy_vote", "x",
                     "presence", "posterior", "winner_idx", "g_lpp",
                     "g_winner", "g_winner_presence", "g_soft_winner",
                     "g_soft_winner_presence", "g_posterior",
                     "g_mixing_log_prob", "g_mixing_logit", "gvote", "gscale",
                     "gvote_presence", "gx", "gpresence", "gdummy_partial"),
                    (vote, scale, vp, dummy_vote, x, presence, post, widx,
                     *gin, gvote, gscale, gvp, gx, gpres, gdummy)):
                setattr(k, name, None if t is None else t.data_ptr())
            k.B, k.O, k.M = B, O, M
            _lib.call("scae_render_gmm_sums_bwd_likelihood_f32",
                      ctypes.byref(pending.desc), *pending.ptrs,
                      ctypes.byref(k), _stream(vote))
        else:
            if pending is not None:
                pending.launch_alone()
            _lib.call("scae_capsule_likelihood_bwd_f32", _p(vote), _p(scale),
                      _p(vp), _p(dummy_vote), _p(x), _p(presence), _p(post),
                      _p(widx), *[_p(g) for g in gin], _p(gvote), _p(gscale),
                      _p(gvp), _p(gx), _p(gpres), _p(gdummy), B, O, M,
                      _stream(vote))
        g_dummy = None
        if g_w is not None or g_s is not None:
            g_dummy = _sum_rows(gdummy.view(B, -1), [ctx.dummy_shape])[0]
        return gvote, gscale, gvp, g_dummy, gx, gpres, None


def capsule_likelihood(vote, scale, vote_presence, dummy_vote, x,
                       presence=None, defer_sum=False):
    return _CapsuleLikelihood.apply(vote, scale, vote_presence, dummy_vote, x,
                                    presence, defer_sum)


_SPARSITY_TYPES = {"l2": 0, "entropy": 1, "kl": 2}


def loss_tail_supported(B, O, n_classes):
    return bool(_lib.load().scae_loss_tail_supported(B, O, n_classes or 0))


class _LossTail(torch.autograd.Function):
    @_fwd
    def forward(ctx, lpp, posterior, caps_presence, cls_w, cls_b, label,
                rec_sums, reg, cfg):
        _need_hip(lpp, posterior, caps_presence, cls_w, cls_b, rec_sums, reg)
        ctx.slots = (_slot(cls_w, ctx), _slot(cls_b, ctx))
        lpp, posterior, caps_presence = _c(lpp), _c(posterior), _c(caps_presence)
        cls_w, cls_b, label = _c(cls_w), _c(cls_b), _c(label)
        rec_sums, reg = _c(rec_sums), _c(reg)
        B, O1, M = posterior.shape
        O = O1 - 1
        ncls = 0 if cls_w is None else cls_w.shape[0]
        (n_classes_cfg, prior_type, post_type, sparsity_on, weights,
         within_const, w_reg) = cfg
        w5 = (ctypes.c_float * 5)(*weights)
        ints = (B, O, M, ncls, int(n_classes_cfg or 0), prior_type, post_type,
                int(sparsity_on))
        both = torch.empty(16, device=lpp.device, dtype=lpp.dtype)
        out = both[:12]
        wc = float("nan") if within_const is None else float(within_const)
        lab = None if label is None else ctypes.c_void_p(label.data_ptr())
        ex = _lib.LossExtras()
        if rec_sums is not None:
            ex.rec_sums, ex.n_rec = rec_sums.data_ptr(), rec_sums.numel()
        if reg is not None:
            ex.reg, ex.w_reg = reg.data_ptr(), float(w_reg)
        loss = both[12]
        ex.loss = loss.data_ptr()
        defer = ctx.plan.fused and rec_sums is not None and \
            any(ctx.needs_input_grad) and \
            bool(_lib.load().scae_loss_tail_defer_preferred(B, O))
        ev = ctx.plan.evaluation if ctx.plan.fused and rec_sums is not None else None
        if ev is not None and label is not None and not ctx.plan.holds("class_probs"):
            ev = None
        defer = defer and ev is None
        tl = ctx.plan.train_log if ctx.plan.fused and rec_sums is not None and ev is None \
            else None
        if tl is not None and label is not None and not ctx.plan.holds("class_probs"):
            tl = None
        ex.defer_combine = int(defer or ev is not None)
        ws = torch.empty(_lib.load().scae_loss_tail_workspace_floats(
            ints[0], ints[1], ints[3]), device=lpp.device, dtype=lpp.dtype)
        tail = (_p(lpp), _p(posterior), _p(caps_presence), _p(cls_w), _p(cls_b),
                lab, ctypes.byref(ex), _p(out), _p(ws), *ints, w5, wc)
        parked = ctx.plan.take("class_probs")
        if tl is not None:
            probs = (None, None) if label is None else parked.keep[4:6]
            ex.train_log = ctypes.pointer(tl.fused_desc(*probs, label))
        if ev is not None and parked is not None and ev.sink is not None:
            ev.sink_written = True
            _lib.call("scae_loss_tail_fwd_class_probs_sink_f32", *tail, *parked.args,
                      ctypes.c_void_p(ev.sink.ptr), _stream(lpp))
        elif parked is not None:
            _lib.call("scae_loss_tail_fwd_class_probs_f32", *tail, *parked.args,
                      _stream(lpp))
        else:
            _lib.call("scae_loss_tail_fwd_f32", *tail, _stream(lpp))
        if ev is not None:
            probs = (None, None) if label is None else parked.keep[4:6]
            ev.fused_launch(tail, *probs, keep=(ws, both, ex, w5), stream_ref=lpp)
        ctx.save_for_backward(lpp, posterior, caps_presence, ws,
                              *([cls_w, cls_b, label] if label is not None
                                else []),
                              *([rec_sums] if rec_sums is not None else []),
                              *([reg] if reg is not None else []))
        ctx.has = (label is not None, rec_sums is not None, reg is not None)
        ctx.call = (ints, tuple(weights), wc, float(w_reg))
        ctx.set_materialize_grads(False)
        ctx.deferred = None
        if defer:
            ctx.deferred = _PendingCombine(
                tail, (lpp, posterior, caps_presence, cls_w, cls_b, label,
                       rec_sums, reg, ws, w5, both, ex), loss.data_ptr(),
                out.data_ptr(), lpp)
            ctx.plan.park("combine", ctx.deferred)
        return loss, out

    @_bwd
    def backward(ctx, g_loss, gout):
        saved = list(ctx.saved_tensors)
        lpp, posterior, cp, ws = saved[:4]
        rest = saved[4:]
        has_label, has_rec, has_reg = ctx.has
        cls_w = cls_b = label = rec_sums = reg = None
        if has_label:
            cls_w, cls_b, label = rest[:3]
            rest = rest[3:]
        if has_rec:
            rec_sums, rest = rest[0], rest[1:]
        if has_reg:
            reg = rest[0]
        ints, weights, wc, w_reg = ctx.call
        g_lpp, g_post, g_cp = (torch.empty_like(t) for t in (lpp, posterior, cp))
        g_w = _grad_out(ctx.slots[0], cls_w) if cls_w is not None else None
        g_b = _grad_out(ctx.slots[1], cls_b) if cls_b is not None else None
        g_rec = torch.empty_like(rec_sums) if has_rec else None
        g_reg = torch.empty_like(reg) if has_reg else None
        ex = _lib.LossExtras()
        if has_rec:
            ex.rec_sums, ex.n_rec = rec_sums.data_ptr(), rec_sums.numel()
            ex.g_rec_sums = g_rec.data_ptr()
        if has_reg:
            ex.reg, ex.w_reg, ex.g_reg = reg.data_ptr(), w_reg, g_reg.data_ptr()
        if g_loss is None and gout is None:
            gout = torch.zeros(12, device=lpp.device, dtype=lpp.dtype)
        if g_loss is not None:
            g_loss = g_loss.contiguous()
            ex.g_loss = g_loss.data_ptr()
        pend = ctx.deferred
        if pend is not None and ctx.plan.holds("combine", pend):
            ctx.plan.take("combine")
            ex.defer_combine, ex.loss, ex.out12 = 1, pend.loss_ptr, pend.out_ptr
            ex.train_log = pend.keep[-1].train_log
        w5 = (ctypes.c_float * 5)(*weights)
        lab = None if label is None else ctypes.c_void_p(label.data_ptr())
        _lib.call("scae_loss_tail_bwd_f32", _p(lpp), _p(posterior), _p(cp),
                  _p(cls_w), _p(cls_b), lab, ctypes.byref(ex),
                  _p(_c(gout)), _p(ws), _p(g_lpp), _p(g_post), _p(g_cp),
                  _p(g_w), _p(g_b), *ints, w5, wc, _stream(lpp))
        return g_lpp, g_post, g_cp, g_w, g_b, None, g_rec, g_reg, None


def loss_tail_scalar(lpp, posterior, caps_presence, cls_w, cls_b, label,
                     n_classes, prior_type, post_type, sparsity_on, weights,
                     within_const=None, rec_sums=None, reg=None, w_reg=0.):
    if label is None:
        cls_w = cls_b = None
    cfg = (n_classes, _SPARSITY_TYPES[prior_type], _SPARSITY_TYPES[post_type],
           bool(sparsity_on), [float(w) for w in weights], within_const,
           float(w_reg))
    return _LossTail.apply(lpp, posterior, caps_presence, cls_w, cls_b, label,
                           rec_sums, reg, cfg)


class EvalEpilogue:

    def __init__(self, device):
        self.acc = torch.zeros(_lib.EVAL_ACC_DOUBLES, device=device, dtype=torch.float64)
        self.batch3 = torch.zeros(3, device=device, dtype=torch.float32)
        self.fused = False
        self._keep = None
        self.sink = None
        self.sink_written = False
        self.records = None
        self.records_alone = False

    def fused_launch(self, tail, prior, post, keep, stream_ref):
        _need_hip(prior, post)
        sink = ctypes.c_void_p(self.sink.ptr) if self.sink_written else None
        records = None
        if self.records is not None:
            records = ctypes.c_void_p(self.records.ptr)
            self.records_alone = False
        _lib.call("scae_eval_tail_records_f32", *tail, _p(prior), _p(post), _p(self.acc),
                  _p(self.batch3), sink, records, _stream(stream_ref))
        self.fused, self._keep = True, (keep, prior, post)

    def accumulate(self, loss, out12, prior, post, label):
        _need_hip(loss, out12, prior, post)
        B = 1 if label is None else label.shape[0]
        ncls = 0 if prior is None else prior.shape[-1]
        loss, out12, prior, post = _c(loss), _c(out12), _c(prior), _c(post)
        lab = None if label is None else ctypes.c_void_p(_c(label).data_ptr())
        _lib.call("scae_eval_accumulate_f32", _p(loss), _p(out12), _p(prior), _p(post), lab,
                  B, ncls, _p(self.acc), _p(self.batch3), _stream(loss))
        self._keep = (loss, out12, prior, post, label)


class _EvalRows:

    def __init__(self, device, int64s):
        self.desc = torch.zeros(int64s, device=device, dtype=torch.int64)
        self.ptr = self.desc.data_ptr()
        self.rows = None

    def _check(self, rows, shape_ok, what):
        if rows.dtype != torch.float32 or not shape_ok or not rows.is_contiguous() \
                or rows.device != self.desc.device:
            raise ValueError(what)

    def _set(self, rows, *more):
        self.rows = rows
        head = [0, 0] if rows is None else [rows.data_ptr(), rows.shape[0]]
        self.desc.copy_(torch.tensor(head + [0, 0, *more], dtype=torch.int64))

    def off(self):
        self.point(None)

    def status(self):
        v = self.desc[2:4].cpu()
        return int(v[0]), bool(v[1])


class EvalSink(_EvalRows):

    def __init__(self, device):
        super().__init__(device, _lib.EVAL_SINK_INT64S)

    def point(self, rows):
        if rows is not None:
            self._check(rows, rows.dim() == 3 and rows.shape[1] == 2, "sink rows must be a "
                        "contiguous (N, 2, O) fp32 tensor on the sink's device")
        self._set(rows)

    def launch_alone(self, caps_presence, posterior):
        _need_hip(caps_presence, posterior)
        cp, post = _c(caps_presence.detach()), _c(posterior.detach())
        B, O1, M = post.shape
        _lib.call("scae_eval_features_f32", _p(cp), _p(post), B, O1 - 1, M,
                  ctypes.c_void_p(self.ptr), _stream(cp))
        self._keep = (cp, post)


class EvalRecords(_EvalRows):

    def __init__(self, device):
        super().__init__(device, _lib.EVAL_RECORDS_INT64S)
        self.confusion = None

    def point(self, rows, confusion=None, labelled=True):
        R = _lib.EVAL_RECORD_FLOATS
        if rows is None:
            confusion = None
        else:
            self._check(rows, rows.dim() == 2 and rows.shape[1] == R,
                        f"records rows must be a contiguous (N, {R}) fp32 tensor on the "
                        "records' device")
            if confusion is not None and (
                    confusion.dtype != torch.int64 or confusion.dim() != 3
                    or confusion.shape[0] != 2 or confusion.shape[1] != confusion.shape[2]
                    or not confusion.is_contiguous() or confusion.device != self.desc.device):
                raise ValueError("confusion must be a contiguous (2, ncls, ncls) int64 tensor "
                                 "on the records' device")
        self.confusion = confusion
        self._set(rows, 0 if confusion is None else confusion.data_ptr(),
                  0 if confusion is None else confusion.shape[1], int(bool(labelled)))

    def launch_alone(self, prior, post, label, lpp, rec_sums=None, rec_pixels=None):
        _need_hip(prior, post, lpp, rec_sums, rec_pixels)
        prior, post, label, lpp = (_c(t.detach()) if t is not None else None
                                   for t in (prior, post, label, lpp))
        rec = rec_sums if rec_sums is not None else rec_pixels
        rec = _c(rec.detach()).flatten(1) if rec is not None else None
        B, M = lpp.shape
        ncls = 0 if prior is None else prior.shape[-1]
        lab = None if label is None else ctypes.c_void_p(label.data_ptr())
        _lib.call("scae_eval_records_f32", _p(prior), _p(post), lab, _p(lpp),
                  _p(rec if rec_sums is not None else None),
                  _p(rec if rec_sums is None else None), B, ncls, M,
                  0 if rec is None else rec.shape[1], ctypes.c_void_p(self.ptr), _stream(lpp))
        self._keep = (prior, post, label, lpp, rec)


TRAIN_LOG_INDEX = {"loss": 0, "accuracy": 1, "prior_accuracy": 2, "posterior_accuracy": 3,
                   "log_prob": 5, "prior_within_sparsity_loss": 6,
                   "prior_between_sparsity_loss": 7, "posterior_within_sparsity_loss": 8,
                   "posterior_between_sparsity_loss": 9, "prior_cls_xe": 10,
                   "posterior_cls_xe": 11, "rec_ll": 12, "rec_ll_loss": 13,
                   "log_prob_loss": 14, "cpr_dynamic_reg_loss": 15, "learning_rate": 16,
                   "mse": 17, "part_caps_loss": 18}


def ring_order(count, capacity):
    k = min(count, capacity)
    steps = list(range(count - k, count))
    return [s % capacity for s in steps], steps


class TrainLog:

    def __init__(self, capacity, device, lr=None):
        self.capacity = int(capacity)
        self.rows = torch.zeros(self.capacity, _lib.TRAIN_LOG_ROW, device=device,
                                dtype=torch.float32)
        self.step = torch.zeros(1, device=device, dtype=torch.int64)
        self.acc = torch.zeros(_lib.EVAL_ACC_DOUBLES, device=device, dtype=torch.float64)
        self.lr = lr
        self.count = 0
        self.fused = False
        self._keep = None

    def _desc(self, prior, post, label):
        d = _lib.TrainLogDesc()
        d.rows, d.step, d.acc = self.rows.data_ptr(), self.step.data_ptr(), \
            self.acc.data_ptr()
        d.capacity = self.capacity
        d.lr = None if self.lr is None else self.lr.data_ptr()
        if label is not None:
            d.prior_prob, d.post_prob, d.label = prior.data_ptr(), post.data_ptr(), \
                label.data_ptr()
            d.ncls = prior.shape[-1]
        return d

    def fused_desc(self, prior, post, label):
        _need_hip(prior, post)
        d = self._desc(prior, post, label)
        self.fused, self._keep = True, (d, prior, post, label)
        return d

    def log_alone(self, loss, out12, extra2, prior, post, label):
        _need_hip(loss, out12, extra2, prior, post)
        loss, out12, extra2 = _c(loss), _c(out12), _c(extra2)
        prior, post, label = _c(prior), _c(post), _c(label)
        B = 1 if label is None else label.shape[0]
        d = self._desc(prior, post, label)
        _lib.call("scae_train_log_f32", _p(loss), _p(out12), _p(extra2), ctypes.byref(d), B,
                  _stream(loss))
        self._keep = (d, loss, out12, extra2, prior, post, label)

    def reset(self):
        self.rows.zero_()
        self.step.zero_()
        self.acc.zero_()
        self.count = 0


def loss_tail(*args, **kwargs):
    return loss_tail_scalar(*args, **kwargs)[1]


class DecoderInputs:

    FIELDS = ("templates", "templates_alpha", "pose", "presence", "bg_image",
              "bg_value", "bg_mixing_logit", "temperature_logit", "out_scale")

    def __init__(self, output_size, **tensors):
        self.output_size = tuple(output_size)
        for f in self.FIELDS:
            setattr(self, f, tensors.get(f))

    def tensors(self):
        return [getattr(self, f) for f in self.FIELDS]


def _make_desc(tensors, output_size):
    (templates, alpha, pose, presence, bg_image, bg_value, bg_ml, temp,
     out_scale) = tensors
    B0, M, C, th, tw = templates.shape
    B = pose.shape[0]
    if B % B0:
        raise ValueError(f"{B} poses cannot share {B0} template sets")
    H, W = output_size
    d = DecoderDesc(_p(templates), _p(alpha), _p(pose), _p(presence),
                    _p(bg_image), _p(bg_value), _p(bg_ml), _p(temp),
                    _p(out_scale), B, M, C, th, tw, H, W, B // B0)
    return d, (B, M, C, th, tw, H, W)


def _decoder_backward(ctx_tensors, output_size, needs, x, lse_post, lse_prior,
                      g_lp, g_tt, g_ml, g_tile=None, slots=None,
                      alpha_shape=None, park=False):
    (templates, alpha, pose, presence, bg_image, bg_value, bg_ml, temp,
     out_scale) = ctx_tensors
    d, (B, M, C, th, tw, H, W) = _make_desc(ctx_tensors, output_size)
    dev, dt = templates.device, templates.dtype
    g_templates = torch.empty_like(templates)
    g_alpha_p = torch.empty(B, M, th, tw, device=dev, dtype=dt) \
        if alpha is not None else None
    g_pose = torch.empty_like(pose)
    g_presence = torch.empty_like(presence) if presence is not None else None
    g_bg_image = torch.empty_like(bg_image) if bg_image is not None else None
    g_scal = torch.empty(B, M + 1, 4, device=dev, dtype=dt)
    slots = slots or [None] * 9
    jobs, g_alpha, gs = [], None, [None] * 4
    if alpha is not None:
        ashape = tuple(alpha_shape or alpha.shape)
        jobs.append(dict(partial=g_alpha_p.view(B, -1), shapes=[ashape],
                         outs=[_grad_out(slots[1], alpha, ashape)],
                         defer=slots[1] is not None))
    scal = [(i, t) for i, t in enumerate((bg_value, bg_ml, temp, out_scale))
            if t is not None]
    if scal:
        jobs.append(dict(partial=g_scal.view(-1, 4),
                         shapes=[t.shape for _, t in scal],
                         starts=[i for i, _ in scal],
                         outs=[_grad_out(slots[5 + i], t) for i, t in scal],
                         defer=all(slots[5 + i] is not None
                                   for i, _ in scal)))
    if park:
        plan = _plan()
        park = plan.deferred is not None and all(
            job["defer"] and all(_in_slot(o) for o in job["outs"])
            for job in jobs)
    if g_tile is not None and park:
        plan.flush_scope("deferring")
        addr = lambda t: None if t is None else t.data_ptr()
        plan.park("k1_bwd", _PendingK1Backward(
            d, ctx_tensors, (x, lse_post, lse_prior, g_tile),
            (addr(g_templates), g_alpha_p, addr(g_pose), addr(g_presence),
             addr(g_bg_image), g_scal), templates))
    elif g_tile is not None:
        _lib.call("scae_render_gmm_sums_bwd_f32", ctypes.byref(d), _p(x),
                  _p(lse_post), _p(lse_prior), _p(g_tile), _p(g_templates),
                  _p(g_alpha_p), _p(g_pose), _p(g_presence), _p(g_bg_image),
                  _p(g_scal), _stream(templates))
    else:
        _lib.call("scae_render_gmm_bwd_f32", ctypes.byref(d), _p(x),
                  _p(lse_post), _p(lse_prior), _p(g_lp), _p(g_tt), _p(g_ml),
                  _p(g_templates), _p(g_alpha_p), _p(g_pose), _p(g_presence),
                  _p(g_bg_image), _p(g_scal), _stream(templates))
    res = _sum_rows_multi(jobs) if jobs else []
    if alpha is not None:
        g_alpha = res[0][0]
    if scal:
        for (i, _), o in zip(scal, res[-1]):
            gs[i] = o
    return (g_templates, g_alpha, g_pose, g_presence, g_bg_image, *gs)


def _prep_decoder(tensors):
    _need_hip(*tensors)
    tensors = [_c(_detached(t)) for t in tensors]
    if tensors[1] is not None:
        tensors[1] = tensors[1].reshape(-1, *tensors[1].shape[-2:])
    return tensors


class _RenderTemplates(torch.autograd.Function):

    @_fwd
    def forward(ctx, output_size, *tensors):
        t = _prep_decoder(tensors)
# ... 393 lines not shown
```

### torch_scae_amd/step_plan.py

```python
import collections
import contextlib
import contextvars
import weakref

ANY = "*"
_LIVE = weakref.WeakSet()


class Ride:

    __slots__ = ("carriers", "readers", "scope", "abi", "what")

    def __init__(self, what, carriers, readers=(), scope="deferring", abi=""):
        self.what, self.carriers, self.readers = what, tuple(carriers), readers
        self.scope, self.abi = scope, abi


RIDES = collections.OrderedDict([
    ("tc_fwd", Ride(
        "the colour MLP's forward (K10)",
        carriers=("_PartEncoder.forward",), scope="offer",
        abi="scae_capsule_head_conv_fwd_tc_f32")),
    ("logprob_fwd", Ride(
        "the reconstruction likelihood's forward (K1)",
        carriers=("_SetEncoder.forward",), scope="offer",
        abi="scae_set_encoder_fwd_logprob_f32")),
    ("trunk_bwd", Ride(
        "the object encoder trunk's backward (K2b), set by set behind the "
        "output attention's",
        carriers=("_SeedAttention.backward",), scope="offer",
        abi="scae_object_encoder_bwd_gemm_f32")),
    ("class_probs", Ride(
        "SCAE.forward's two classifier heads (one wave per image)",
        carriers=("_LossTail.forward",), scope="fusing",
        abi="scae_loss_tail_fwd_class_probs_f32")),
    ("combine", Ride(
        "the loss tail's batch combine (one workgroup)",
        carriers=("_LossTail.backward",), scope="fusing",
        abi="scae_loss_tail_bwd_f32 (scae_loss_extras.defer_combine)")),
    ("k1_bwd", Ride(
        "the reconstruction likelihood's backward (K1)",
        carriers=("_CapsuleLikelihood.backward",), readers=ANY,
        abi="scae_render_gmm_sums_bwd_likelihood_f32")),
    ("wgrads", Ride(
        "the capsule MLPs' four weight-gradient GEMMs",
        carriers=("_SeedAttention.backward",),
        abi="scae_seed_attention_mfma_bwd_gemm_f32")),
    ("tc_bwd", Ride(
        "the colour MLP's backward (K10)",
        carriers=("_PartEncoder.backward",),
        readers=("_CapsuleHead.backward",),
        abi="scae_capsule_head_bwd_tc_f32")),
    ("reduce", Ride(
        "the output attention's partial-row reduction",
        carriers=("_PartEncoder.backward", "_ConvStack.backward"),
        abi="scae_conv3x3_bwd_pair_reduce_f32")),
    ("fold_bwd", Ride(
        "the folding products' backward (K2d)",
        carriers=("_PartEncoder.backward", "_ConvStack.backward"),
        abi="scae_conv3x3_bwd_pair_fold_f32")),
])


class StepPlan:
    def __init__(self, name="step", prologue=None):
        _LIVE.add(self)
        self.name = name
        self.target = None
        self.rider = None
        self.offers = {}
        self.parked = {}
        self.deferred = None
        self.sums_to_optimizer = False
        self.held_sums = []
        self.prologue = prologue
        self.bf16 = False
        self.carry_trunk_bwd = True
        self.noise = {}
        self.noise_salt = 0
        self.side_stream = None
        self.evaluation = None
        self.train_log = None

    @contextlib.contextmanager
    def active(self):
        token = _CURRENT.set(self)
        try:
            yield self
        finally:
            _CURRENT.reset(token)

    @property
    def fused(self):
        return self.target is not None

    @property
    def parking(self):
        return self.target is not None and self.deferred is not None

    def offer(self, kind, work):
        assert RIDES[kind].scope == "offer", kind
        self.offers[kind] = work

    def claim(self, kind):
        return self.offers.pop(kind, None)

    def park(self, kind, work):
        assert kind in RIDES and RIDES[kind].scope != "offer", kind
        stale = self.parked.pop(kind, None)
        if stale is not None:
            stale.launch_alone()
        self.parked[kind] = work

    def take(self, kind):
        return self.parked.pop(kind, None)

    def holds(self, kind, work=None):
        held = self.parked.get(kind)
        return held is not None and (work is None or held is work)

    def flush(self, *kinds):
        for kind in RIDES:
            if (not kinds or kind in kinds) and kind in self.parked:
                self.parked.pop(kind).launch_alone()

    def flush_scope(self, scope):
        self.flush(*[k for k, r in RIDES.items() if r.scope == scope])

    def enter(self, node):
        if not self.parked:
            return
        for kind in RIDES:
            if kind not in self.parked:
                continue
            ride = RIDES[kind]
            if node in ride.carriers:
                continue
            if ride.readers == ANY or node in ride.readers:
                self.parked.pop(kind).launch_alone()

    def flush_sums(self):
        if self.deferred:
            units = list(self.deferred)
            del self.deferred[:]
            from . import ops
            ops._launch_sum_units(units)

    def take_held_sums(self):
        units, self.held_sums = self.held_sums, []
        return units

    @contextlib.contextmanager
    def fusing(self, target):
        prev = (self.target, self.rider)
        self.target, self.rider = target, None
        self.parked.clear()
        self.offers.clear()
        ok = False
        try:
            yield self
            ok = True
        finally:
            self.target, self.rider = prev
            self.offers.clear()
            if ok:
                self.flush_scope("fusing")

    @contextlib.contextmanager
    def deferring(self):
        outer = self.deferred
        if outer is None:
            self.deferred = []
        ok = False
        try:
            yield self
            ok = True
        finally:
            if outer is None:
                try:
                    if ok:
                        self.flush_scope("deferring")
                        if self.sums_to_optimizer:
                            self.held_sums.extend(self.deferred)
                            del self.deferred[:]
                        else:
                            self.flush_sums()
                finally:
                    self.deferred = None

    @contextlib.contextmanager
    def with_prologue(self, pro):
        prev, self.prologue = self.prologue, pro
        try:
            yield pro
        finally:
            self.prologue = prev

    @contextlib.contextmanager
    def evaluating(self, epilogue):
        prev, self.evaluation = self.evaluation, epilogue
        try:
            yield self
        finally:
            self.evaluation = prev

    @contextlib.contextmanager
    def logging(self, train_log):
        prev, self.train_log = self.train_log, train_log
        try:
            yield self
        finally:
            self.train_log = prev

    @contextlib.contextmanager
    def precision(self, bf16):
        prev, self.bf16 = self.bf16, bool(bf16)
        try:
            yield self
        finally:
            self.bf16 = prev


def live_plans():
    return list(_LIVE)


_CURRENT = contextvars.ContextVar("scae_step_plan", default=None)
ambient = StepPlan("ambient")


def current():
    plan = _CURRENT.get()
    return ambient if plan is None else plan


@contextlib.contextmanager
def running(plan, node):
    token = _CURRENT.set(plan)
    try:
        plan.enter(node)
        yield plan
    finally:
        _CURRENT.reset(token)
```

Baseline: 270,000.

## Fuse capsule votes backward into the likelihood backward kernel launch

Adds a votes_bwd ride so the capsule votes' backward is computed inside the capsule likelihood backward kernel, image by image, via a new votes descriptor pointer in the likelihood bwd struct. The votes backward then reuses the just-produced vote gradients instead of launching a separate kernel and rereading them from memory. Identity checks on pointers, versions and shapes confirm the carried results match the gradients autograd later delivers, and the code falls back to the separate launch if the kernel reports unsupported. The device code is refactored into shared helpers (caps_eval, bwd_vote, bwd_caps) using fma-based dot products, and the standalone kernel is rewritten to use them. The added bookkeeping brings Python overhead and a risk of stale or mismatched gradients.

```diff
diff --git a/include/scae_hip.h b/include/scae_hip.h
--- a/include/scae_hip.h
+++ b/include/scae_hip.h
@@ -838,6 +838,7 @@
       *g_posterior, *g_mixing_log_prob, *g_mixing_logit;
   float *gvote, *gscale, *gvote_presence, *gx, *gpresence, *gdummy_partial;
   int B, O, M;
+  const scae_votes_desc *votes;
 } scae_likelihood_bwd_desc;
 int scae_render_gmm_sums_bwd_likelihood_f32(
     const scae_decoder_desc *d, const float *x, const float *lse_post, const float *lse_prior,
diff --git a/torch_scae_amd/_lib.py b/torch_scae_amd/_lib.py
--- a/torch_scae_amd/_lib.py
+++ b/torch_scae_amd/_lib.py
@@ -113,8 +113,10 @@
 def check(rc, what):
     if rc != 0:
         msg = load().scae_error_string(rc)
-        raise ScaeHipError(f"{what} failed with code {rc}: "
+        err = ScaeHipError(f"{what} failed with code {rc}: "
                            f"{msg.decode() if msg else '?'}")
+        err.code = rc
+        raise err
 
 
 def call(name, *args):
diff --git a/torch_scae_amd/csrc/capsule_votes.hip b/torch_scae_amd/csrc/capsule_votes.hip
--- a/torch_scae_amd/csrc/capsule_votes.hip
+++ b/torch_scae_amd/csrc/capsule_votes.hip
@@ -73,96 +73,29 @@
   }
 }
 
-__global__ __launch_bounds__(NT) void votes_bwd_kernel(
-    VoteArgs a, const float *__restrict__ gvote, const float *__restrict__ gscale,
-    const float *__restrict__ gvp, const float *__restrict__ glc,
-    const float *__restrict__ glv, const float *__restrict__ greg,
-    float *__restrict__ gall, float *__restrict__ gcpr_in,
-    const float *__restrict__ g_caps_presence, const int *__restrict__ caps_arg,
-    float *__restrict__ gall_gated) {
+__global__ __launch_bounds__(NT) void votes_bwd_kernel(VoteArgs a, VoteGrads w) {
   const int bo = blockIdx.x, o = bo % a.O, V = a.V, lane = threadIdx.x;
   const float *ap = a.all_param + (size_t)bo * a.ldp;
-  float *ga = gall + (size_t)bo * a.ldp;
-  float *gg = gall_gated ? gall_gated + (size_t)bo * a.ldp : nullptr;
-  auto put = [&](int i, float v) {
-    ga[i] = v;
-    if (gg) gg[i] = ap[i] > 0.f ? v : 0.f;
+  auto put = [&](int col, float v) {
+    w.gall[(size_t)bo * a.ldp + col] = v;
+    if (w.gall_gated) w.gall_gated[(size_t)bo * a.ldp + col] = ap[col] > 0.f ? v : 0.f;
   };
-
-  float cv[6];
+  const float reg_w = w.greg ? w.greg[0] / (float)a.B : 0.f;
+  Xf C;
+  float pc;
+  caps_eval(a, ap, bo, o, C, pc);
+  float sum[7] = {0.f, 0.f, 0.f, 0.f, 0.f, 0.f, 0.f};
+  for (int v0 = 0; v0 < V; v0 += NT) {
+    float part[7] = {0.f, 0.f, 0.f, 0.f, 0.f, 0.f, 0.f};
+    if (v0 + lane < V) bwd_vote(a, w, ap, bo, o, v0 + lane, C.o, pc, reg_w, put, part);
+    for (int j = 0; j < NT / 4; ++j) {
 #pragma unroll
-  for (int i = 0; i < 6; ++i) cv[i] = ap[6 * V + i] + a.bias_cvr[o * 6 + i];
-  Xf C;
-  xf_eval(cv, a.similarity, C);
-  float lc = ap[6 * V + 6] + a.bias_caps[o];
-  if (a.noise_caps) lc += (a.noise_caps[bo] - 0.5f) * a.noise_scale;
-  const float pc = scae::sigmoidf_(lc);
-  const float reg_w = greg ? greg[0] / (float)a.B : 0.f;
-
-  float gC[6] = {0, 0, 0, 0, 0, 0};
-  float gpc = 0.f;
-  for (int v = lane; v < V; v += NT) {
-    float pr[6], dyn[6];
-#pragma unroll
-    for (int i = 0; i < 6; ++i) {
-      dyn[i] = a.allow_deformations ? ap[v * 6 + i] : 0.f;
-      pr[i] = dyn[i] + a.cpr_static[((size_t)o * V + v) * 6 + i];
+      for (int k = 0; k < 7; ++k) sum[k] += __shfl(part[k], (lane & 3) + 4 * j, 64);
     }
-    Xf P;
-    xf_eval(pr, a.similarity, P);
-    float gv[6] = {0, 0, 0, 0, 0, 0};
-    if (gvote) {
-#pragma unroll
-      for (int i = 0; i < 6; ++i) gv[i] = gvote[((size_t)bo * V + v) * 6 + i];
-    }
-    gC[0] += gv[0] * P.o[0] + gv[1] * P.o[1] + gv[2] * P.o[2];
-    gC[1] += gv[0] * P.o[3] + gv[1] * P.o[4] + gv[2] * P.o[5];
-    gC[2] += gv[2];
-    gC[3] += gv[3] * P.o[0] + gv[4] * P.o[1] + gv[5] * P.o[2];
-    gC[4] += gv[3] * P.o[3] + gv[4] * P.o[4] + gv[5] * P.o[5];
-    gC[5] += gv[5];
-    float gP[6];
-    gP[0] = gv[0] * C.o[0] + gv[3] * C.o[3];
-    gP[1] = gv[1] * C.o[0] + gv[4] * C.o[3];
-    gP[2] = gv[2] * C.o[0] + gv[5] * C.o[3];
-    gP[3] = gv[0] * C.o[1] + gv[3] * C.o[4];
-    gP[4] = gv[1] * C.o[1] + gv[4] * C.o[4];
-    gP[5] = gv[2] * C.o[1] + gv[5] * C.o[4];
-    float gin[6];
-    xf_backward(P, a.similarity, gP, gin);
-#pragma unroll
-    for (int i = 0; i < 6; ++i) {
-      gcpr_in[((size_t)bo * V + v) * 6 + i] = gin[i];
-      put(v * 6 + i, a.allow_deformations ? gin[i] + reg_w * dyn[i] : 0.f);
-    }
-
-    float lv = ap[6 * V + 7 + v] + a.bias_vote[o * V + v];
-    if (a.noise_vote) lv += (a.noise_vote[(size_t)bo * V + v] - 0.5f) * a.noise_scale;
-    const float pv = scae::sigmoidf_(lv);
-    float g_vp = gvp ? gvp[(size_t)bo * V + v] : 0.f;
-    if (g_caps_presence && caps_arg[bo] == v) g_vp += g_caps_presence[bo];
-    gpc += g_vp * pv;
-    float g_lv = g_vp * pc * pv * (1.f - pv);
-    if (glv) g_lv += glv[(size_t)bo * V + v];
-    put(6 * V + 7 + v, g_lv);
-    float g_sc = 0.f;
-    if (a.learn_vote_scale && gscale)
-      g_sc = gscale[(size_t)bo * V + v] *
-             scae::softplus_grad(ap[7 * V + 7 + v] + a.bias_scale[o * V + v] + .5f);
-    put(7 * V + 7 + v, g_sc);
   }
 #pragma unroll
-  for (int i = 0; i < 6; ++i) gC[i] = scae::wave_sum(gC[i]);
-  gpc = scae::wave_sum(gpc);
-  if (lane == 0) {
-    float gin[6];
-    xf_backward(C, a.similarity, gC, gin);
-#pragma unroll
-    for (int i = 0; i < 6; ++i) put(6 * V + i, gin[i]);
-    float g_lc = gpc * pc * (1.f - pc);
-    if (glc) g_lc += glc[bo];
-    put(6 * V + 6, g_lc);
-  }
+  for (int k = 0; k < 7; ++k) sum[k] = quad_sum(sum[k]);
+  if (lane == 0) bwd_caps(a, w, ap, bo, o, sum, put);
 }
 
 int check_votes(const VoteArgs &a) {
@@ -209,8 +142,8 @@
   int rc = check_votes(a);
   if (rc) return rc;
   SCAE_REQUIRE(gall_param && gcpr_in && (!gcaps_presence || caps_arg));
-  scae::launch(votes_bwd_kernel, dim3(B * O), dim3(NT), 0, (hipStream_t)stream, a,
-                     gvote, gscale, gvote_presence, glogit_caps, glogit_vote, greg,
-                     gall_param, gcpr_in, gcaps_presence, caps_arg, gall_param_gated);
+  VoteGrads w{gvote, gscale, gvote_presence, glogit_caps, glogit_vote, greg, gcaps_presence,
+              caps_arg, gall_param, gcpr_in, gall_param_gated};
+  scae::launch(votes_bwd_kernel, dim3(B * O), dim3(NT), 0, (hipStream_t)stream, a, w);
   return scae_launch_status();
 }
diff --git a/torch_scae_amd/csrc/capsule_votes_dev.h b/torch_scae_amd/csrc/capsule_votes_dev.h
--- a/torch_scae_amd/csrc/capsule_votes_dev.h
+++ b/torch_scae_amd/csrc/capsule_votes_dev.h
@@ -3,6 +3,17 @@
 
 namespace scae_votes {
 constexpr float kTwoPi = 6.283185307179586f;
+
+__device__ __forceinline__ float ps2(float a0, float b0, float a1, float b1) {
+  return fmaf(a1, b1, a0 * b0);
+}
+__device__ __forceinline__ float ps3(float a0, float b0, float a1, float b1, float a2, float b2) {
+  return fmaf(a2, b2, fmaf(a1, b1, a0 * b0));
+}
+__device__ __forceinline__ float ps4(float a0, float b0, float a1, float b1, float a2, float b2,
+                                     float a3, float b3) {
+  return fmaf(a3, b3, fmaf(a2, b2, fmaf(a1, b1, a0 * b0)));
+}
 
 struct Xf {
   float sx, sy, sh, c, s, tx, ty;
@@ -19,9 +30,9 @@
   g.sh = tanhf(p[3] * 5.f);
   g.tx = tanhf(p[4] * 5.f);
   g.ty = tanhf(p[5] * 5.f);
-  g.dsh = 5.f * (1.f - g.sh * g.sh);
-  g.dtx = 5.f * (1.f - g.tx * g.tx);
-  g.dty = 5.f * (1.f - g.ty * g.ty);
+  g.dsh = 5.f * fmaf(-g.sh, g.sh, 1.f);
+  g.dtx = 5.f * fmaf(-g.tx, g.tx, 1.f);
+  g.dty = 5.f * fmaf(-g.ty, g.ty, 1.f);
   const float th = p[2] * kTwoPi;
   g.c = cosf(th);
   g.s = sinf(th);
@@ -33,8 +44,9 @@
     g.o[4] = g.sx * g.c;
     g.o[5] = g.ty;
   } else {
-    g.o[0] = g.sx * g.c + g.sh * g.sy * g.s;
-    g.o[1] = -g.sx * g.s + g.sh * g.sy * g.c;
+    const float hy = g.sh * g.sy;
+    g.o[0] = ps2(g.sx, g.c, hy, g.s);
+    g.o[1] = ps2(-g.sx, g.s, hy, g.c);
     g.o[2] = g.tx;
     g.o[3] = g.sy * g.s;
     g.o[4] = g.sy * g.c;
@@ -46,16 +58,17 @@
                                             float *gp) {
   float gsx, gsy, gsh, gth;
   if (similarity) {
-    gsx = go[0] * g.c - go[1] * g.s + go[3] * g.s + go[4] * g.c;
+    gsx = ps4(go[0], g.c, -go[1], g.s, go[3], g.s, go[4], g.c);
     gsy = 0.f;
     gsh = 0.f;
-    gth = g.sx * (-go[0] * g.s - go[1] * g.c + go[3] * g.c - go[4] * g.s);
+    gth = g.sx * ps4(-go[0], g.s, -go[1], g.c, go[3], g.c, -go[4], g.s);
   } else {
-    gsx = go[0] * g.c - go[1] * g.s;
-    gsy = go[0] * g.sh * g.s + go[1] * g.sh * g.c + go[3] * g.s + go[4] * g.c;
-    gsh = go[0] * g.sy * g.s + go[1] * g.sy * g.c;
-    gth = go[0] * (-g.sx * g.s + g.sh * g.sy * g.c) +
-          go[1] * (-g.sx * g.c - g.sh * g.sy * g.s) + go[3] * g.sy * g.c - go[4] * g.sy * g.s;
+    const float hy = g.sh * g.sy;
+    gsx = ps2(go[0], g.c, -go[1], g.s);
+    gsy = ps4(go[0] * g.sh, g.s, go[1] * g.sh, g.c, go[3], g.s, go[4], g.c);
+    gsh = ps2(go[0] * g.sy, g.s, go[1] * g.sy, g.c);
+    gth = ps4(go[0], ps2(-g.sx, g.s, hy, g.c), go[1], ps2(-g.sx, g.c, -hy, g.s), go[3] * g.sy,
+              g.c, -go[4] * g.sy, g.s);
   }
   gp[0] = gsx * g.dsx;
   gp[1] = gsy * g.dsy;
@@ -160,6 +173,103 @@
   }
 }
 
+
+__device__ __forceinline__ void caps_eval(const VoteArgs &a, const float *ap, int bo, int o,
+                                          Xf &C, float &pc) {
+  const int V = a.V;
+  float cv[6];
+#pragma unroll
+  for (int k = 0; k < 6; ++k) cv[k] = ap[6 * V + k] + a.bias_cvr[o * 6 + k];
+  xf_eval(cv, a.similarity, C);
+  float lc = ap[6 * V + 6] + a.bias_caps[o];
+  if (a.noise_caps) lc = fmaf(a.noise_caps[bo] - 0.5f, a.noise_scale, lc);
+  pc = scae::sigmoidf_(lc);
+}
+
+template <class Put>
+__device__ __forceinline__ void bwd_vote(const VoteArgs &a, const VoteGrads &w, const float *ap,
+                                         int bo, int o, int v, const float *Co, float pc,
+                                         float reg_w, Put put, float (&part)[7]) {
+  const int V = a.V;
+  float pr[6], dyn[6];
+#pragma unroll
+  for (int k = 0; k < 6; ++k) {
+    dyn[k] = a.allow_deformations ? ap[v * 6 + k] : 0.f;
+    pr[k] = dyn[k] + a.cpr_static[((size_t)o * V + v) * 6 + k];
+  }
+  Xf P;
+  xf_eval(pr, a.similarity, P);
+  float gv[6] = {0, 0, 0, 0, 0, 0};
+  if (w.gvote) {
+#pragma unroll
+    for (int k = 0; k < 6; ++k) gv[k] = w.gvote[((size_t)bo * V + v) * 6 + k];
+  }
+  part[0] = ps3(gv[0], P.o[0], gv[1], P.o[1], gv[2], P.o[2]);
+  part[1] = ps3(gv[0], P.o[3], gv[1], P.o[4], gv[2], P.o[5]);
+  part[2] = gv[2];
+  part[3] = ps3(gv[3], P.o[0], gv[4], P.o[1], gv[5], P.o[2]);
+  part[4] = ps3(gv[3], P.o[3], gv[4], P.o[4], gv[5], P.o[5]);
+  part[5] = gv[5];
+  float gP[6];
+  gP[0] = ps2(gv[0], Co[0], gv[3], Co[3]);
+  gP[1] = ps2(gv[1], Co[0], gv[4], Co[3]);
+  gP[2] = ps2(gv[2], Co[0], gv[5], Co[3]);
+  gP[3] = ps2(gv[0], Co[1], gv[3], Co[4]);
+  gP[4] = ps2(gv[1], Co[1], gv[4], Co[4]);
+  gP[5] = ps2(gv[2], Co[1], gv[5], Co[4]);
+  float gin[6];
+  xf_backward(P, a.similarity, gP, gin);
+#pragma unroll
+  for (int k = 0; k < 6; ++k) {
+    w.gcpr_in[((size_t)bo * V + v) * 6 + k] = gin[k];
+    put(v * 6 + k, a.allow_deformations ? fmaf(reg_w, dyn[k], gin[k]) : 0.f);
+  }
+  float lv = ap[6 * V + 7 + v] + a.bias_vote[o * V + v];
+  if (a.noise_vote) lv = fmaf(a.noise_vote[(size_t)bo * V + v] - 0.5f, a.noise_scale, lv);
+  const float pv = scae::sigmoidf_(lv);
+  float g_vp = w.gvp ? w.gvp[(size_t)bo * V + v] : 0.f;
+  if (w.g_caps_presence && w.caps_arg[bo] == v) g_vp += w.g_caps_presence[bo];
+  part[6] = g_vp * pv;
+  const float qv = 1.f - pv, t_lv = g_vp * pc * pv;
+  float g_lv = w.glv ? fmaf(t_lv, qv, w.glv[(size_t)bo * V + v]) : t_lv * qv;
+  put(6 * V + 7 + v, g_lv);
+  float g_sc = 0.f;
+  if (a.learn_vote_scale && w.gscale)
+    g_sc = w.gscale[(size_t)bo * V + v] *
+           scae::softplus_grad(ap[7 * V + 7 + v] + a.bias_scale[o * V + v] + .5f);
+  put(7 * V + 7 + v, g_sc);
+}
+
+template <class Put>
+__device__ __forceinline__ void bwd_caps(const VoteArgs &a, const VoteGrads &w, const float *ap,
+                                         int bo, int o, const float *sum, Put put) {
+  const int V = a.V;
+  float gC[6], gpc = sum[6];
+#pragma unroll
+  for (int k = 0; k < 6; ++k) gC[k] = sum[k];
+  Xf C;
+  float pc;
+  caps_eval(a, ap, bo, o, C, pc);
+  float gin[6];
+  xf_backward(C, a.similarity, gC, gin);
+#pragma unroll
+  for (int k = 0; k < 6; ++k) put(6 * V + k, gin[k]);
+  const float qc = 1.f - pc, t_lc = gpc * pc;
+  float g_lc = w.glc ? fmaf(t_lc, qc, w.glc[bo]) : t_lc * qc;
+  put(6 * V + 6, g_lc);
+}
+
+__device__ __forceinline__ float quarter_sum(const float *part7, int V, int k, int quarter) {
+  float t = 0.f;
+  for (int v = quarter; v < V; v += 4) t += part7[(size_t)v * 7 + k];
+  return t;
+}
+__device__ __forceinline__ float quad_sum(float t) {
+  t += __shfl_xor(t, 1, 64);
+  t += __shfl_xor(t, 2, 64);
+  return t;
+}
+
 template <int NTH>
 __device__ __forceinline__ void bwd_block(const VoteArgs &a, const VoteGrads &w, float *grows,
                                           int ld, float *red, int b0, int o) {
@@ -177,61 +287,11 @@
     if (b < a.B) {
       const int bo = b * a.O + o;
       const float *ap = a.all_param + (size_t)bo * a.ldp;
-      float cv[6];
-#pragma unroll
-      for (int k = 0; k < 6; ++k) cv[k] = ap[6 * V + k] + a.bias_cvr[o * 6 + k];
       Xf C;
-      xf_eval(cv, a.similarity, C);
-      float lc = ap[6 * V + 6] + a.bias_caps[o];
-      if (a.noise_caps) lc += (a.noise_caps[bo] - 0.5f) * a.noise_scale;
-      const float pc = scae::sigmoidf_(lc);
-      float pr[6], dyn[6];
-#pragma unroll
-      for (int k = 0; k < 6; ++k) {
-        dyn[k] = a.allow_deformations ? ap[v * 6 + k] : 0.f;
-        pr[k] = dyn[k] + a.cpr_static[((size_t)o * V + v) * 6 + k];
-      }
-      Xf P;
-      xf_eval(pr, a.similarity, P);
-      float gv[6] = {0, 0, 0, 0, 0, 0};
-      if (w.gvote) {
-#pragma unroll
-        for (int k = 0; k < 6; ++k) gv[k] = w.gvote[((size_t)bo * V + v) * 6 + k];
-      }
-      part[0] = gv[0] * P.o[0] + gv[1] * P.o[1] + gv[2] * P.o[2];
-      part[1] = gv[0] * P.o[3] + gv[1] * P.o[4] + gv[2] * P.o[5];
-      part[2] = gv[2];
-      part[3] = gv[3] * P.o[0] + gv[4] * P.o[1] + gv[5] * P.o[2];
-      part[4] = gv[3] * P.o[3] + gv[4] * P.o[4] + gv[5] * P.o[5];
-      part[5] = gv[5];
-      float gP[6];
-      gP[0] = gv[0] * C.o[0] + gv[3] * C.o[3];
-      gP[1] = gv[1] * C.o[0] + gv[4] * C.o[3];
-      gP[2] = gv[2] * C.o[0] + gv[5] * C.o[3];
-      gP[3] = gv[0] * C.o[1] + gv[3] * C.o[4];
-      gP[4] = gv[1] * C.o[1] + gv[4] * C.o[4];
-      gP[5] = gv[2] * C.o[1] + gv[5] * C.o[4];
-      float gin[6];
-      xf_backward(P, a.similarity, gP, gin);
-#pragma unroll
-      for (int k = 0; k < 6; ++k) {
-        w.gcpr_in[((size_t)bo * V + v) * 6 + k] = gin[k];
-        put(ap, i, bo, v * 6 + k, a.allow_deformations ? gin[k] + reg_w * dyn[k] : 0.f);
-      }
-      float lv = ap[6 * V + 7 + v] + a.bias_vote[o * V + v];
-      if (a.noise_vote) lv += (a.noise_vote[(size_t)bo * V + v] - 0.5f) * a.noise_scale;
-      const float pv = scae::sigmoidf_(lv);
-      float g_vp = w.gvp ? w.gvp[(size_t)bo * V + v] : 0.f;
-      if (w.g_caps_presence && w.caps_arg[bo] == v) g_vp += w.g_caps_presence[bo];
-      part[6] = g_vp * pv;
-      float g_lv = g_vp * pc * pv * (1.f - pv);
-      if (w.glv) g_lv += w.glv[(size_t)bo * V + v];
-      put(ap, i, bo, 6 * V + 7 + v, g_lv);
-      float g_sc = 0.f;
-      if (a.learn_vote_scale && w.gscale)
-        g_sc = w.gscale[(size_t)bo * V + v] *
-               scae::softplus_grad(ap[7 * V + 7 + v] + a.bias_scale[o * V + v] + .5f);
-      put(ap, i, bo, 7 * V + 7 + v, g_sc);
+      float pc;
+      caps_eval(a, ap, bo, o, C, pc);
+      bwd_vote(a, w, ap, bo, o, v, C.o, pc, reg_w,
+               [&](int col, float val) { put(ap, i, bo, col, val); }, part);
     }
 #pragma unroll
     for (int k = 0; k < 7; ++k) red[(size_t)e * 7 + k] = part[k];
@@ -240,10 +300,8 @@
   {
     float t = 0.f;
     const int i = tid >> 5, k = (tid >> 2) & 7, part = tid & 3;
-    if (tid < 512 && k < 7)
-      for (int v = part; v < V; v += 4) t += red[(size_t)(i * V + v) * 7 + k];
-    t += __shfl_xor(t, 1, 64);
-    t += __shfl_xor(t, 2, 64);
+    if (tid < 512 && k < 7) t = quarter_sum(red + (size_t)i * V * 7, V, k, part);
+    t = quad_sum(t);
     __syncthreads();
     if (tid < 512 && k < 7 && part == 0) red[i * 8 + k] = t;
   }
@@ -253,24 +311,8 @@
     if (b < a.B) {
       const int bo = b * a.O + o;
       const float *ap = a.all_param + (size_t)bo * a.ldp;
-      float gC[6], gpc = red[i * 8 + 6];
-#pragma unroll
-      for (int k = 0; k < 6; ++k) gC[k] = red[i * 8 + k];
-      float cv[6];
-#pragma unroll
-      for (int k = 0; k < 6; ++k) cv[k] = ap[6 * V + k] + a.bias_cvr[o * 6 + k];
-      Xf C;
-      xf_eval(cv, a.similarity, C);
-      float lc = ap[6 * V + 6] + a.bias_caps[o];
-      if (a.noise_caps) lc += (a.noise_caps[bo] - 0.5f) * a.noise_scale;
-      const float pc = scae::sigmoidf_(lc);
-      float gin[6];
-      xf_backward(C, a.similarity, gC, gin);
-#pragma unroll
-      for (int k = 0; k < 6; ++k) put(ap, i, bo, 6 * V + k, gin[k]);
-      float g_lc = gpc * pc * (1.f - pc);
-      if (w.glc) g_lc += w.glc[bo];
-      put(ap, i, bo, 6 * V + 6, g_lc);
+      bwd_caps(a, w, ap, bo, o, red + i * 8,
+               [&](int col, float val) { put(ap, i, bo, col, val); });
     } else {
       for (int col = 0; col < A; ++col) grows[i * ld + col] = 0.f;
     }
@@ -282,4 +324,58 @@
   }
   __syncthreads();
 }
-}
+
+__host__ __device__ inline int image_scratch_floats(int V) { return 7 * V + 16; }
+
+template <int NTH>
+__device__ __forceinline__ void bwd_image(const VoteArgs &a, const VoteGrads &w, float *red,
+                                          int cap, int b) {
+  const int V = a.V, O = a.O, tid = threadIdx.x;
+  const float reg_w = w.greg ? w.greg[0] / (float)a.B : 0.f;
+  int oc = cap / image_scratch_floats(V);
+  oc = oc < O ? oc : O;
+  float *sums = red + (size_t)oc * V * 7;
+  auto put = [&](const float *ap, int bo, int col, float v) {
+    w.gall[(size_t)bo * a.ldp + col] = v;
+    if (w.gall_gated) w.gall_gated[(size_t)bo * a.ldp + col] = ap[col] > 0.f ? v : 0.f;
+  };
+  for (int o0 = 0; o0 < O; o0 += oc) {
+    const int n = O - o0 < oc ? O - o0 : oc;
+    for (int i = tid; i < n; i += NTH) {
+      const int o = o0 + i, bo = b * O + o;
+      Xf C;
+      float pc;
+      caps_eval(a, a.all_param + (size_t)bo * a.ldp, bo, o, C, pc);
+#pragma unroll
+      for (int k = 0; k < 6; ++k) sums[i * 16 + 8 + k] = C.o[k];
+      sums[i * 16 + 14] = pc;
+    }
+    __syncthreads();
+    for (int e = tid; e < n * V; e += NTH) {
+      const int i = e / V, v = e - i * V, o = o0 + i, bo = b * O + o;
+      const float *ap = a.all_param + (size_t)bo * a.ldp;
+      float part[7];
+      bwd_vote(a, w, ap, bo, o, v, sums + i * 16 + 8, sums[i * 16 + 14], reg_w,
+               [&](int col, float val) { put(ap, bo, col, val); }, part);
+#pragma unroll
+      for (int k = 0; k < 7; ++k) red[(size_t)e * 7 + k] = part[k];
+    }
+    __syncthreads();
+    for (int t0 = 0; t0 < n * 32; t0 += NTH) {
+      const int it = t0 + tid, i = it >> 5, k = (it >> 2) & 7, part = it & 3;
+      float t = 0.f;
+      if (i < n && k < 7) t = quarter_sum(red + (size_t)i * V * 7, V, k, part);
+      t = quad_sum(t);
+      if (i < n && k < 7 && part == 0) sums[i * 16 + k] = t;
+    }
+    __syncthreads();
+    for (int i = tid; i < n; i += NTH) {
+      const int o = o0 + i, bo = b * O + o;
+      const float *ap = a.all_param + (size_t)bo * a.ldp;
+      bwd_caps(a, w, ap, bo, o, sums + i * 16,
+               [&](int col, float val) { put(ap, bo, col, val); });
+    }
+    if (o0 + oc < O) __syncthreads();
+  }
+}
+}
diff --git a/torch_scae_amd/csrc/render_bwd_likelihood.hip b/torch_scae_amd/csrc/render_bwd_likelihood.hip
--- a/torch_scae_amd/csrc/render_bwd_likelihood.hip
+++ b/torch_scae_amd/csrc/render_bwd_likelihood.hip
@@ -1,5 +1,6 @@
 #include "common.h"
 #include "capsule_likelihood_dev.h"
+#include "capsule_votes_dev.h"
 #include "render_gmm_wave_dev.h"
 
 namespace {
@@ -9,6 +10,9 @@
   const float *g_lpp, *g_winner, *g_winner_presence, *g_soft_winner, *g_soft_winner_presence,
       *g_posterior, *g_mlp, *g_mlogit;
   float *gvote, *gscale, *gvp, *gx, *gpresence, *gdummy;
+  int votes, lds_floats;
+  scae_votes::VoteArgs va;
+  scae_votes::VoteGrads vg;
 };
 
 template <int C>
@@ -25,6 +29,12 @@
         lk.a, lk.winner_idx, lk.g_lpp, lk.g_winner, lk.g_winner_presence, lk.g_soft_winner,
         lk.g_soft_winner_presence, lk.g_posterior, lk.g_mlp, lk.g_mlogit, lk.gvote, lk.gscale,
         lk.gvp, lk.gx, lk.gpresence, lk.gdummy, smem, blockIdx.x, n_lk);
+    if (lk.votes) {
+      for (int b = blockIdx.x; b < lk.a.B; b += n_lk) {
+        __syncthreads();
+        scae_votes::bwd_image<256>(lk.va, lk.vg, smem, lk.lds_floats, b);
+      }
+    }
     return;
   }
   const int id = (int)blockIdx.x - n_lk, K = d.M + 1, b = id / K, k = id - b * K;
@@ -37,7 +47,8 @@
 int launch(const scae_decoder_desc *d, const scae_k1::CellGeom &g, const scae_k1::LpTiling &lt,
            const float *x, const float *lse_post, const float *lse_prior, const float *g_tile,
            float *g_templates, float *g_alpha_partial, float *g_pose, float *g_presence,
-           float *g_bg_image, float *g_scalar_partial, const LkBwd &lk, hipStream_t st) {
+           float *g_bg_image, float *g_scalar_partial, LkBwd lk, bool riders_only,
+           hipStream_t st) {
   const size_t lds_k = scae_lk::lk_lds(lk.a.O, lk.a.M, true);
   const size_t lds = g.lds > lds_k ? g.lds : lds_k;
   if (lds > 48 * 1024) {
@@ -47,7 +58,9 @@
     if (e != hipSuccess) return (int)e;
   }
   const int n_lk = lk.a.B < 1024 ? lk.a.B : 1024;
-  scae::launch((bwd_cell_likelihood_kernel<C>), dim3(n_lk + (d->M + 1) * d->B), dim3(256),
+  lk.lds_floats = (int)(lds / sizeof(float));
+  const int n_k1 = riders_only ? 0 : (d->M + 1) * d->B;
+  scae::launch((bwd_cell_likelihood_kernel<C>), dim3(n_lk + n_k1), dim3(256),
                      lds, st, *d, x, lse_post, lse_prior, g_tile, lt.tiles, lt.ppb, g_templates,
                      g_alpha_partial, g_pose, g_presence, g_bg_image, g_scalar_partial,
                      g.chunk_rows, g.max_items, g.item_budget, lk, n_lk);
@@ -63,10 +76,21 @@
   SCAE_REQUIRE(d && k);
   const char *e = getenv("SCAE_FUSE_K1_K4_BWD");
   const scae_k1::CellGeom g = scae_k1::cell_geom(d);
-  const bool fits = !(e && *e == '0') && g.lds && (d->C == 1 || d->C == 3) && k->O <= 64 &&
-                    scae_lk::lk_lds(k->O, k->M, true) <= g.lds && k->B > 0 && k->O > 0 &&
-                    k->M > 0 && d->template_repeat <= 1;
-  if (!fits) {
+  const scae_votes_desc *v = k->votes;
+  const bool merge = !(e && *e == '0');
+  const bool shapes =
+      g.lds && (d->C == 1 || d->C == 3) && k->O <= 64 &&
+      scae_lk::lk_lds(k->O, k->M, true) <= g.lds && k->B > 0 && k->O > 0 && k->M > 0 &&
+      d->template_repeat <= 1 &&
+      (!v || (size_t)scae_votes::image_scratch_floats(k->M) * sizeof(float) <= g.lds);
+  const bool fits = merge && shapes;
+  if (v) {
+    SCAE_REQUIRE(v->all_param && v->cpr_static && v->bias_cvr && v->bias_caps && v->bias_vote &&
+                 v->bias_scale && v->gall_param && v->gcpr_in && v->V == k->M &&
+                 v->ld_param >= 8 * v->V + 7 && (!v->gcaps_presence || v->caps_arg));
+    if (!shapes) return SCAE_ERR_UNSUPPORTED;
+  }
+  if (!fits && !v) {
     int rc = scae_render_gmm_sums_bwd_f32(d, x, lse_post, lse_prior, g_tile_sums, g_templates,
                                           g_alpha_partial, g_pose, g_presence, g_bg_image,
                                           g_scalar_partial, stream);
@@ -100,12 +124,31 @@
            k->gvote_presence,
            k->gx,
            k->gpresence,
-           k->gdummy_partial};
+           k->gdummy_partial,
+           v != nullptr,
+           0,
+           {},
+           {}};
+  if (v) {
+    lk.va = scae_votes::VoteArgs{v->all_param, v->cpr_static, v->bias_cvr, v->bias_caps,
+                                 v->bias_vote, v->bias_scale, v->noise_caps, v->noise_vote,
+                                 v->noise_scale, k->B, k->O, v->V, v->similarity,
+                                 v->learn_vote_scale, v->allow_deformations, v->ld_param};
+    lk.vg = scae_votes::VoteGrads{k->gvote, k->gscale, k->gvote_presence, v->glogit_caps,
+                                  v->glogit_vote, v->greg, v->gcaps_presence, v->caps_arg,
+                                  v->gall_param, v->gcpr_in, v->gall_param_gated};
+  }
   hipStream_t st = (hipStream_t)stream;
+  if (!merge) {
+    int rc = scae_render_gmm_sums_bwd_f32(d, x, lse_post, lse_prior, g_tile_sums, g_templates,
+                                          g_alpha_partial, g_pose, g_presence, g_bg_image,
+                                          g_scalar_partial, stream);
+    if (rc) return rc;
+  }
   return d->C == 1 ? launch<1>(d, g, lt, x, lse_post, lse_prior, g_tile_sums, g_templates,
                                g_alpha_partial, g_pose, g_presence, g_bg_image, g_scalar_partial,
-                               lk, st)
+                               lk, !merge, st)
                    : launch<3>(d, g, lt, x, lse_post, lse_prior, g_tile_sums, g_templates,
                                g_alpha_partial, g_pose, g_presence, g_bg_image, g_scalar_partial,
-                               lk, st);
+                               lk, !merge, st);
 }
diff --git a/torch_scae_amd/ops.py b/torch_scae_amd/ops.py
--- a/torch_scae_amd/ops.py
+++ b/torch_scae_amd/ops.py
@@ -2116,29 +2116,31 @@
                                          b_scale)]
         ctx.set_materialize_grads(False)
         ctx.mark_non_differentiable(reg)
+        ctx.votes_ride = None
+        if ctx.plan.fused and ctx.plan.carry_votes_bwd and \
+                any(ctx.needs_input_grad):
+            ctx.votes_ride = step_plan.VotesBackwardRide(vote, scale, vp)
+            ctx.votes_ride.node = ctx
+            ctx.plan.offer("votes_bwd", ctx.votes_ride)
         return vote, scale, vp, lc, lv, reg_loss, caps_presence, reg
 
-    @_bwd
-    def backward(ctx, gvote, gscale, gvp, glc, glv, greg, gcp, _greg_partial):
-        ones_flags, has_bias, noise_scale, (V, ldp, sim, lvs, adef) = ctx.meta
+    @staticmethod
+    def votes_backward_desc(ctx, grads):
+        ones_flags, _, noise_scale, (V, ldp, sim, lvs, adef) = ctx.meta
         L = len(ones_flags)
         saved = list(ctx.saved_tensors)
         x, caps_arg = saved[0], saved[1]
-        weights = saved[2:2 + L]
-        acts = saved[2 + L:2 + 2 * L]
+        all_param = saved[1 + 2 * L]
         rest = saved[2 + 2 * L:]
         vargs = rest[:5]
         rest = rest[5:]
         noise_caps = rest.pop(0) if ctx.has_noise[0] else None
         noise_vote = rest.pop(0) if ctx.has_noise[1] else None
-        all_param = acts[-1]
         B, O, A = all_param.shape
-        dev, dt = x.device, x.dtype
-        padded = lambda: torch.empty(B, O, ldp, device=dev,
-                                     dtype=dt)[:, :, :A]
+        padded = lambda: torch.empty(B, O, ldp, device=x.device,
+                                     dtype=x.dtype)[:, :, :A]
         gall, ggated = padded(), padded()
-        gin = torch.empty(B, O, V, 6, device=dev, dtype=dt)
-        grads = [_c(g) for g in (gvote, gscale, gvp, glc, glv, greg, gcp)]
+        gin = torch.empty(B, O, V, 6, device=x.device, dtype=x.dtype)
         v = _lib.VotesDesc()
         for name, t in zip(("all_param", "cpr_static", "bias_cvr", "bias_caps",
                             "bias_vote", "bias_scale", "noise_caps",
@@ -2153,6 +2155,25 @@
         v.caps_arg = caps_arg.data_ptr()
         v.gall_param, v.gcpr_in, v.gall_param_gated = \
             gall.data_ptr(), gin.data_ptr(), ggated.data_ptr()
+        return v, (gall, ggated, gin), (saved, grads)
+
+    @_bwd
+    def backward(ctx, gvote, gscale, gvp, glc, glv, greg, gcp, _greg_partial):
+        ones_flags, has_bias, noise_scale, (V, ldp, sim, lvs, adef) = ctx.meta
+        L = len(ones_flags)
+        saved = list(ctx.saved_tensors)
+        x = saved[0]
+        weights = saved[2:2 + L]
+        acts = saved[2 + L:2 + 2 * L]
+        vargs = saved[2 + 2 * L:7 + 2 * L]
+        B, O, A = acts[-1].shape
+        grads = [_c(g) for g in (gvote, gscale, gvp, glc, glv, greg, gcp)]
+        ride, ctx.votes_ride = ctx.votes_ride, None
+        carried = ride.claim(grads) if ride is not None else None
+        if carried is not None:
+            v, (gall, ggated, gin) = None, carried
+        else:
+            v, (gall, ggated, gin), _ = _ChainVotes.votes_backward_desc(ctx, grads)
         gx, gws, gbs = _chain_backward(
             x, weights, acts, ones_flags, has_bias, False, ctx.slots, True,
             gpre=ggated, votes=v,
@@ -2317,6 +2338,9 @@
         ctx.save_for_backward(*saved)
         ctx.has_presence = presence is not None
         ctx.dims = (B, O, M)
+        ride = ctx.plan.claim("votes_bwd")
+        ctx.votes_ride = ride if ride is not None and \
+            ride.feeds(vote, scale, vp) else None
         ctx.dummy_shape = dummy_vote.shape
         ctx.mark_non_differentiable(binary, widx, from_caps)
         ctx.set_materialize_grads(False)
@@ -2358,9 +2382,29 @@
                      *gin, gvote, gscale, gvp, gx, gpres, gdummy)):
                 setattr(k, name, None if t is None else t.data_ptr())
             k.B, k.O, k.M = B, O, M
-            _lib.call("scae_render_gmm_sums_bwd_likelihood_f32",
-                      ctypes.byref(pending.desc), *pending.ptrs,
-                      ctypes.byref(k), _stream(vote))
+            args = (ctypes.byref(pending.desc), *pending.ptrs, ctypes.byref(k),
+                    _stream(vote))
+            ride, carried = ctx.votes_ride, False
+            if ride is not None and ride.wanted(ctx.plan):
+                g_cp, g_reg = ctx.plan.tail_grads or (None, None)
+                read = [gvote, gscale, gvp, None, None, g_reg, g_cp]
+                v, results, keep = _ChainVotes.votes_backward_desc(ride.node, read)
+                k.votes = ctypes.pointer(v)
+                try:
+                    _lib.call("scae_render_gmm_sums_bwd_likelihood_f32", *args)
+                    carried = True
+                except ScaeHipError as err:
+                    if getattr(err, "code", None) != _lib.ERR_UNSUPPORTED:
+                        raise
+                if carried:
+                    ride.carried(read, results)
+                    k._keep = (v, results, keep)
+                else:
+                    ride.declined()
+                    k.votes = None
+            ctx.plan.tail_grads = None
+            if not carried:
+                _lib.call("scae_render_gmm_sums_bwd_likelihood_f32", *args)
         else:
             if pending is not None:
                 pending.launch_alone()
@@ -2507,6 +2551,7 @@
                   _p(cls_w), _p(cls_b), lab, ctypes.byref(ex),
                   _p(_c(gout)), _p(ws), _p(g_lpp), _p(g_post), _p(g_cp),
                   _p(g_w), _p(g_b), *ints, w5, wc, _stream(lpp))
+        ctx.plan.tail_grads = (g_cp, g_reg)
         return g_lpp, g_post, g_cp, g_w, g_b, None, g_rec, g_reg, None
 
 
diff --git a/torch_scae_amd/step_plan.py b/torch_scae_amd/step_plan.py
--- a/torch_scae_amd/step_plan.py
+++ b/torch_scae_amd/step_plan.py
@@ -30,6 +30,12 @@
         "output attention's",
         carriers=("_SeedAttention.backward",), scope="offer",
         abi="scae_object_encoder_bwd_gemm_f32")),
+    ("votes_bwd", Ride(
+        "the capsule votes' backward (K3), image by image behind the capsule "
+        "likelihood's",
+        carriers=("_CapsuleLikelihood.backward",), scope="offer",
+        abi="scae_render_gmm_sums_bwd_likelihood_f32 "
+            "(scae_likelihood_bwd_desc.votes)")),
     ("class_probs", Ride(
         "SCAE.forward's two classifier heads (one wave per image)",
         carriers=("_LossTail.forward",), scope="fusing",
@@ -62,6 +68,43 @@
 ])
 
 
+def _ident(t):
+    if t is None:
+        return None
+    return (t.data_ptr(), t.numel(), t.dtype, t.is_contiguous(), t._version)
+
+
+class VotesBackwardRide:
+
+    def __init__(self, vote, scale, vote_presence):
+        self.outputs = tuple(_ident(t)[:4] for t in (vote, scale, vote_presence))
+        self.read = None
+        self.results = None
+        self.keep = None
+
+    def feeds(self, vote, scale, vote_presence):
+        return self.outputs == tuple(
+            _ident(t)[:4] for t in (vote, scale, vote_presence))
+
+    def wanted(self, plan):
+        return bool(plan.parking and plan.carry_votes_bwd)
+
+    def carried(self, grads, results):
+        self.keep = tuple(grads)
+        self.read = tuple(_ident(g) for g in grads)
+        self.results = results
+
+    def declined(self):
+        self.read = self.results = self.keep = None
+
+    def claim(self, grads):
+        if self.results is None or \
+                self.read != tuple(_ident(g) for g in grads):
+            return None
+        results, self.results = self.results, None
+        return results
+
+
 class StepPlan:
     def __init__(self, name="step", prologue=None):
         _LIVE.add(self)
@@ -76,6 +119,8 @@
         self.prologue = prologue
         self.bf16 = False
         self.carry_trunk_bwd = True
+        self.carry_votes_bwd = True
+        self.tail_grads = None
         self.noise = {}
         self.noise_salt = 0
         self.side_stream = None
@@ -156,6 +201,7 @@
         self.target, self.rider = target, None
         self.parked.clear()
         self.offers.clear()
+        self.tail_grads = None
         ok = False
         try:
             yield self
@@ -163,6 +209,7 @@
         finally:
             self.target, self.rider = prev
             self.offers.clear()
+            self.tail_grads = None
             if ok:
                 self.flush_scope("fusing")
 
```

New measurement: 267,300. -1.0%, worse.
